# salesforce/ai-economist

Measured on AMD Instinct MI355X. Metric: agent-steps/sec, gather-trade-build 25x25 4-agent batched envs, higher is better.
Workload: dtype u8/i32 state + f64 coin/utility (f32 observations); 1 GPU; C2 BASELINE configs[1]: gather-trade-build 25x25, 4 agents + planner, Build+CDA+Gather+PeriodicBracketTax, 4096 replicas/GPU, uniform random policy, planner not counted; envs_per_gpu=4096, global_envs=4096, n_agents=4, kernel_specialisation=compile time, parallelism=single GPU

## Files before the change

### ai-economist_amd/csrc/aie_capi.hip

```cpp
#include <hip/hip_runtime.h>

#include <cstdio>
#include <cstdlib>
#include <cstring>
#include <vector>

#include "aie_kernels.hip"
#include "aie_kernels_sampler.hip"
#include "aie_kernels_rollout.hip"
#include "aie_kernels_ose.hip"
#include "aie_kernels_saez.hip"
#include "aie_kernels_ppo.hip"
#include "aie_kernels_mlp.hip"
#include "aie_kernels_mlp_bwd.hip"
#include "aie_kernels_covid.hip"
#include "aie_jit.h"
#include "aie_layout_build.h"
#include "aie_trainer_plan.h"

struct aie_env {
  aie_params P{};
  aie_params* d_params;
  aie_tensor_table tt;
  uint8_t* arena;
// ... 73 lines not shown
        for (size_t q = 0; q < off; q += piece) (void)hipMemUnmap(static_cast<char*>(va) + q, piece);
        (void)hipMemAddressFree(va, total);
      }
    }
    (void)hipGetLastError();
  }
  return hipMalloc(&p, bytes) == hipSuccess ? static_cast<uint8_t*>(p) : nullptr;
}
static void aie_arena_free(uint8_t* arena, size_t vmm_total, size_t vmm_piece) {
  if (!arena) return;
  if (vmm_total) {
    for (size_t q = 0; q < vmm_total; q += vmm_piece) (void)hipMemUnmap(arena + q, vmm_piece);
    (void)hipMemAddressFree(arena, vmm_total);
  } else {
    (void)hipFree(arena);
  }
}

__global__ void aie_init_cells_kernel(const aie_params P, uint8_t* __restrict__ arena) {
  const int64_t q = (int64_t)blockIdx.x * blockDim.x + threadIdx.x;
  if (q >= (int64_t)P.E * P.HW) return;
  const int e = (int)(q / P.HW), cell = (int)(q - (int64_t)e * P.HW);
  reinterpret_cast<uint32_t*>(arena + P.a_records + (int64_t)e * P.rec_bytes + P.o_cells)[cell] = 0x00ff0000u;
}

__global__ void aie_set_flags_kernel(const aie_params P, uint8_t* __restrict__ arena,
                                     const uint8_t* __restrict__ flags, int shared) {
  const int64_t q = (int64_t)blockIdx.x * blockDim.x + threadIdx.x;
  if (q >= (int64_t)P.E * P.HW) return;
  const int e = (int)(q / P.HW), cell = (int)(q - (int64_t)e * P.HW);
  uint32_t* w = reinterpret_cast<uint32_t*>(arena + P.a_records + (int64_t)e * P.rec_bytes + P.o_cells) + cell;
  const uint32_t fl = flags[shared ? cell : q];
  *w = (*w & 0x00ffffffu) | (fl << 24);
}

__global__ void __launch_bounds__(64) aie_src_list_kernel(const aie_params* __restrict__ params, uint8_t* __restrict__ arena) {
  const aie_params& P = *params;
  const int e = (int)blockIdx.x, lane = (int)threadIdx.x, HW = P.HW;
  if (!P.o_src_list || e >= P.E) return;
  uint8_t* rec = arena + P.a_records + (int64_t)e * P.rec_bytes;
  const uint8_t* cb = rec + P.o_cells;
  uint16_t* lst = reinterpret_cast<uint16_t*>(rec + P.o_src_list);
  for (int k = lane; k < AIE_SRC_CAP; k += 64) lst[k] = 0;
  int base = 0;
  for (int rs = 0; rs < 2; ++rs) {
    const uint32_t bit = rs == 0 ? AIE_CELL_WOOD_SRC : AIE_CELL_STONE_SRC;
    for (int q0 = 0; q0 < HW; q0 += 64) {
      const int q = q0 + lane;
      const bool on = q < HW && (cb[4 * q + 3] & bit);
      const uint64_t mask = __ballot(on);
      const int slot = base + __popcll(mask & ((1ull << lane) - 1ull));
      if (on && slot < AIE_SRC_CAP) lst[slot] = (uint16_t)(rs * HW + q);
      base += __popcll(mask);
    }
  }
  if (lane == 0) *reinterpret_cast<int32_t*>(rec + P.o_src_n) = base;
}
static int aie_rebuild_src_lists(aie_env* env) {
  if (env->P.c.scenario != AIE_SCN_GTB || !env->P.o_src_list) return AIE_OK;
  hipLaunchKernelGGL(aie_src_list_kernel, dim3((unsigned)env->P.E), dim3(64), 0, 0, env->d_params, env->arena);
  AIE_HIP_CHECK(env, hipGetLastError());
  AIE_HIP_CHECK(env, hipDeviceSynchronize());
  return AIE_OK;
}

static inline int aie_workgroups_per_cu(size_t lds) {
// ... 1008 lines not shown
```

### ai-economist_amd/csrc/aie_gtb_state.h

```cpp
#pragma once
#include "aie_device.h"

namespace aie {
__device__ __forceinline__ bool can_agent_occupy(const Ctx& c, int r, int col, int agent) {
  if (r < 0 || r >= c.P.H || col < 0 || col >= c.P.W) return false;
  const int cell = r * c.P.W + col;
  const uint32_t w = R_CELLS(c)[cell];
  if (AIE_CELL_FLAGS(w) & AIE_CELL_WATER) return false;
  const int o = AIE_CELL_OWNER(w);
  if (!(o < 0 || o == agent)) return false;
  const int occ = c.locmap[cell];
  return occ == 0 || occ == agent + 1;
}

__device__ __forceinline__ void log_event(const Ctx& c, int type, int a1, int a2, int a3, int a4, int a5,
                                          int a6, int a7, int a8, double f) {
  if (c.tid != 0) return;
  const int k = c.srcn[2];
  if (k >= c.R.ev_cap) return;
  int32_t* row = c.ev + 4 + k * AIE_EV_WORDS;
  row[0] = type; row[1] = a1; row[2] = a2; row[3] = a3; row[4] = a4;
  row[5] = a5; row[6] = a6; row[7] = a7; row[8] = a8; row[9] = 0;
  *reinterpret_cast<double*>(row + 10) = f;
  c.srcn[2] = k + 1;
// ... 121 lines not shown
        if (x >= x0 && x < x0 + P.n_sub_p * P.sub_p_dim && (x - x0) / P.sub_p_dim == i) v = (x - x0) % P.sub_p_dim + 1;
      }
    }
    c.act_p[i] = v;
  }
  if (host && P.n_host_p && ap && i < P.n_host_p) {
    const int32_t* a = ap + (int64_t)c.e * P.act_p_width;
    int v;
    if (P.c.multi_action_mode_planner) {
      v = a[P.hp_row[i]];
      if (v < 0 || v > P.hp_dim[i]) { bad_p = true; v = 0; }
    } else {
      const int x = a[0];
      if (x < 0 || x >= P.AP) bad_p = true;
      v = (x >= P.hp_base[i] && x < P.hp_base[i] + P.hp_dim[i]) ? x - P.hp_base[i] + 1 : 0;
    }
    reinterpret_cast<int32_t*>(arena + c.R.a_host_act_p)[(int64_t)c.e * P.n_host_p + i] = v;
  }
  return (__ballot(bad_a) ? AIE_ERR_AGENT_ACTION : 0) | (__ballot(bad_p) ? AIE_ERR_PLANNER_ACTION : 0);
}

__device__ __forceinline__ uint16_t* dirty_list(const Ctx& c) { return reinterpret_cast<uint16_t*>(c.dirty + 4); }
__device__ __forceinline__ void dirty_add_uniform(const Ctx& c, MTL& m, int cell) {
  if (c.tid == 0 && m.dn < AIE_DIRTY_CAP) dirty_list(c)[m.dn] = (uint16_t)cell;
  m.dn += 1;
}
__device__ __forceinline__ void dirty_add_lane(const Ctx& c, int cell) {
  const int s = atomicAdd(&c.dirty[0], 1);
  if (s < AIE_DIRTY_CAP) dirty_list(c)[s] = (uint16_t)cell;
}
__device__ __forceinline__ void dirty_agent_moved(MTL& m, int i) {
  if (i < 32) m.mv0 |= 1u << i; else m.mv1 |= 1u << (i - 32);
}
__device__ __forceinline__ void store_record_step(const Ctx& c, uint8_t* __restrict__ arena, int wave, int nwaves) {
  uint8_t* g = arena + (int64_t)c.e * c.P.rec_bytes;
  uint4* dst = reinterpret_cast<uint4*>(g);
  const uint4* src = reinterpret_cast<const uint4*>(c.rec);
  const int nq = rec_lds_bytes(c.P) >> 4;
  const int cnt = uni(c.dirty[0]);
  const int q0 = (c.P.o_cells == 0 && cnt <= AIE_DIRTY_CAP) ? (4 * c.P.HW) >> 4 : 0;
  for (int q = q0 + wave * AIE_NT + c.tid; q < nq; q += nwaves * AIE_NT) dst[q] = src[q];
  if (wave == nwaves - 1 && q0 > 0 && c.tid < cnt) {
    const int cell = (int)dirty_list(c)[c.tid];
    reinterpret_cast<uint32_t*>(g + c.P.o_cells)[cell] = R_CELLS(c)[cell];
  }
}

}
```

### ai-economist_amd/csrc/aie_kernels.hip

```cpp
#pragma once
#include "aie_gtb_state.h"
#include "aie_gtb_components.h"
#include "aie_gtb_observe.h"
#include "aie_gtb_layoutgen.h"



__device__ __forceinline__ uint32_t glibc_tables_touch(int lane) {
  uint32_t v = 0;
#pragma unroll
  for (int k = 0; k < 2; ++k) {
    const int line = 2 * lane + k;
    const uint8_t* p = line < 48 ? reinterpret_cast<const uint8_t*>(aie_glibc_powlog_tab) + 64 * line
                     : line < 80 ? reinterpret_cast<const uint8_t*>(aie_glibc_exp_tab) + 64 * (line - 48)
                                 : reinterpret_cast<const uint8_t*>(aie_glibc_log_tab) + 64 * (line - 80);
    if (line < 112) v ^= *reinterpret_cast<const volatile uint32_t*>(p);
  }
  return v;
}

__device__ __forceinline__ void step_rewards_and_done(const aie::Ctx& c, uint8_t* __restrict__ arena, const NextActions& next, int skip,
                                                      bool emit = true, bool close = true) {
  using namespace aie;
  float* const rew_log = close ? rew_log_claim(c.R, R_I32(c, o_rew_slot), R_I32(c, o_rew_epoch), c.R.E, c.P.n, c.tid == 0) : nullptr;
// ... 27 lines not shown
#endif
  const int e_blk = replica_of_block((int)blockIdx.x, next.E);
  if (next.e_hi > 0 && (e_blk < next.e_lo || e_blk >= next.e_hi)) return;
  if (LOG && next.mask && !next.mask[e_blk]) return;
  const bool FAST = rng_fast(P);
  const int tid0 = (int)(threadIdx.x & (AIE_NT - 1));
  uint8_t* grec = arena + (int64_t)e_blk * P.rec_bytes;
  uint32_t* gkey = reinterpret_cast<uint32_t*>(grec + P.o_mt);
  const Ctx c = make_ctx(P, R, lds, e_blk, tid0, arena, LOG, skip,
                         SPEC >= 0);
  const bool SHL = shared_src_list(P);
  uint32_t* const draw_w = reinterpret_cast<uint32_t*>(c.stage);
  int draw_cap = stage_window_words(P);
  if (LOG && R.dev_draw_window > 0 && R.dev_draw_window < draw_cap) draw_cap = R.dev_draw_window;
  const int w0_tail_prio = P.n >= 8 ? 2 : 0;
  const bool REW_ON_W1 = FAST && P.n < 8;
  const int ph = LOG ? next.phase : 0;
  const bool HEAD = ph == 0 || (ph & 1), TAIL = ph == 0 || (ph & 2), OBSERVE = ph != 0 && (ph & 4) && !(ph & 2);
  const bool REBASE = OBSERVE && (ph & 8);
  const bool RETAX = OBSERVE && (ph & 16);
  const bool REGEN = TAIL || (ph & 64), EMIT = TAIL || (ph & 128), CLOSE = TAIL || (ph & 256);
  const bool CLOSE_ONLY = CLOSE && !EMIT;
  const int c_lo = ph ? next.comp_lo : 0, c_hi = ph ? next.comp_hi : P.c.n_components;
  constexpr int COMP_UNROLL = (SPEC >= 0 && !LOG) ? AIE_MAX_COMPONENTS : 1;
  if (wid == 0) {
    Agents A;
    A.hist_dirty = 0;
    A.tax_dirty = false;
    int act_err = 0;
    if (!(skip & AIE_DEV_SKIP_ACTION_DECODE)) act_err = decode_actions(c, A, act_a, act_p, arena);
    else A.act = 0;
    if (TRACE && R.dev_trace && c.tid == 0) R.dev_trace[12 * blockIdx.x] = wall_clock64();
    if (TRACE && R.dev_trace && c.tid == 0) R.dev_trace[12 * blockIdx.x + 9] = wall_clock64();
    MT none;
    load_record(c, arena, none, 0, 2, -1);
    __syncthreads();
    if (TRACE && R.dev_trace && c.tid == 0) R.dev_trace[12 * blockIdx.x + 8] = wall_clock64();
    MTL ml{draw_w, 0, 0u, -AIE_MT_N, 0, 0u, 0u, 0, 0, 0, FAST ? reinterpret_cast<uint32_t*>(c.rec + P.o_mt) : gkey, draw_cap, FAST};
    ml.pos = ml.base = uni(*R_I32(c, o_mt_pos));
    ml.avail = ml.cap < AIE_MT_N - ml.pos ? ml.cap : AIE_MT_N - ml.pos;
    if (FAST) {
      const int covered = 128 * ((ml.cap + 127) >> 7) - (ml.pos & 1);
      if (ml.avail > covered) ml.avail = covered;
    }
    agents_load(c, A);
#ifdef AIE_FLAT_FULL
    const bool flat_in_place = false;
#else
    const bool flat_in_place = ph == 0 && uni(*R_I32(c, o_obs_valid)) != 0 && !(skip & AIE_DEV_FLAT_FULL);
#endif
    if (act_err && c.tid == 0) *R_I32(c, o_error_flags) |= act_err;
    bool cda_in_range = ph == 0;
    if (ph != 0)
      for (int k = c_lo; k < c_hi; ++k) cda_in_range |= P.c.components[k] == AIE_COMP_CDA;
    if (P.has_cda && !(skip & AIE_DEV_SKIP_COMPONENTS) && cda_in_range) cda_decay_price_history(c);
    __syncthreads();
    if (c.tid == 0 && HEAD) *R_I32(c, o_timestep) += 1;
    if (c.ev && c.tid == 0) c.srcn[2] = 0;
    __builtin_amdgcn_s_setprio(3);
    if (TRACE && R.dev_trace && c.tid == 0) R.dev_trace[12 * blockIdx.x + 1] = wall_clock64();
    if (!(skip & AIE_DEV_SKIP_COMPONENTS)) {
#pragma unroll COMP_UNROLL
      for (int k = c_lo; k < c_hi; ++k) {
        switch (P.c.components[k]) {
          case AIE_COMP_BUILD: if (!(skip & AIE_DEV_SKIP_BUILD)) build_component_step(c, ml, A); break;
          case AIE_COMP_CDA: if (!(skip & AIE_DEV_SKIP_CDA)) cda_component_step(c, A); break;
          case AIE_COMP_GATHER: if (!(skip & AIE_DEV_SKIP_GATHER)) gather_component_step(c, ml, A); break;
          case AIE_COMP_TAX: if (!(skip & AIE_DEV_SKIP_TAX)) tax_component_step(c, ml, A); break;
          case AIE_COMP_WEALTH_REDISTRIBUTION: wealth_component_step(c, A); break;
          default: break;
        }
// ... 9 lines not shown
      c.dirty[1] = (int32_t)ml.mv0;
      c.dirty[2] = (int32_t)ml.mv1;
      c.dirty[3] = ml.tw;
    }
    if (TRACE && R.dev_trace && c.tid == 0) R.dev_trace[12 * blockIdx.x + 5] = wall_clock64();
    __syncthreads();
    if (w0_tail_prio) __builtin_amdgcn_s_setprio(2);
    if (RETAX && P.has_tax) {
      if (c.tid < P.n) R_F64(c, o_tax_last_coin)[c.tid] = R_F64(c, o_inv_coin)[c.tid] + R_F64(c, o_esc_coin)[c.tid];
      AIE_WSYNC();
    }
    if (!(skip & AIE_DEV_SKIP_FLAT_AND_MASKS) && (EMIT || OBSERVE)) {
      const bool annealed_first = P.has_tax && P.c.tax_annealing && uni(*R_I32(c, o_timestep)) == 1;
      if (flat_in_place && !A.tax_dirty && !annealed_first) update_flat_observations(c, arena, A.hist_dirty);
      else write_flat_observations(c, arena);
    }
    if (TRACE && R.dev_trace && c.tid == 0) R.dev_trace[12 * blockIdx.x + 10] = wall_clock64();
    if (!REW_ON_W1 && (EMIT || CLOSE)) step_rewards_and_done(c, arena, next, skip, EMIT, CLOSE);
    if (REBASE) {
      AIE_WSYNC();
      current_metrics(c);
      AIE_WSYNC();
      if (c.tid <= P.n) R_F64(c, o_util)[c.tid] = scr_part(c)[c.tid];
      AIE_WSYNC();
    }
    if (w0_tail_prio) __builtin_amdgcn_s_setprio(0);
    __syncthreads();
    if (!(skip & AIE_DEV_SKIP_RECORD_STORE)) store_record_step(c, arena, 0, 2);
    if (TRACE && R.dev_trace && c.tid == 0) R.dev_trace[12 * blockIdx.x + 7] = wall_clock64();
  } else {
    MT m;
    mt_init(m, P);
    const int gpos = *reinterpret_cast<const int32_t*>(grec + P.o_mt_pos);
    load_record(c, arena, m, 1, 2, -1);
    if (skip & AIE_DEV_SKIP_DRAW_WINDOW) {}
    else if (FAST) draw_window_publish_fast(draw_w, draw_cap, (uint32_t)uni((int)gkey[0]), (uint32_t)uni((int)gkey[1]), (uint32_t)uni((int)gkey[2]), uni(gpos), c.tid);
    else draw_window_publish_from_hbm(draw_w, draw_cap, gkey, uni(gpos), c.tid);

    if (SPEC >= 0 && const_tables_in_lds(P)) {
      if (P.has_tax && P.c.tax_model == AIE_TAX_MODEL_WRAPPER)
        for (int q = c.tid; q < P.c.tax_n_disc_rates; q += AIE_NT) const_cast<double*>(c.rtab)[q] = R.c.tax_disc_rates[q];
      for (int q = c.tid; q < P.MA; q += AIE_NT) const_cast<uint32_t*>(c.mtab)[q] = P.mask_test[q];
    }
    __syncthreads();
    if (!(skip & AIE_DEV_SKIP_LOCMAP)) rebuild_locmap(c);
    __syncthreads();
    SrcList src;
    src.S = 0;
#pragma unroll
    for (int k = 0; k < AIE_SRC_CAP / AIE_NT; ++k) src.d[k] = 0;
    src = SHL ? src_list_from_arena(c, arena) : src_list_from_record(c, arena);
    const uint32_t warm = glibc_tables_touch(c.tid);
    if (!FAST && !(skip & AIE_DEV_SKIP_GENERATOR_ROWS)) {
#pragma unroll
      for (int j = 0; j < 9; ++j) m.r[j] = gkey[64 * j + c.tid];
      m.r[9] = c.tid < 48 ? gkey[576 + c.tid] : 0u;
    }
    if ((next.a || next.p) && TAIL) {
      const int per_env = P.n * P.act_a_width + P.act_p_width;
      const int st = uni(*R_I32(c, o_sample_t));
      for (int j = c.tid; j < per_env; j += AIE_NT) sample_action_slot(P, next.seed, next.env_offset, (int64_t)st, c.e, j, next.a, next.p);
      if (c.tid == 0) *R_I32(c, o_sample_t) = st + 1;
    }
    asm volatile("" ::"v"(warm));
    __syncthreads();
    if (next.E > 6144) __builtin_amdgcn_s_setprio(0);
    else __builtin_amdgcn_s_setprio(2);
    if (FAST) {
      const uint32_t* st = R_U32(c, o_mt);
      m.fkey = (uint32_t)uni((int)st[0]);
      m.fblk = (uint32_t)uni((int)st[1]);
      m.fsalt = (uint32_t)uni((int)st[2]);
    } else if (uni(c.dirty[3]) != 0) {
      mt_rows_from_hbm(m, gkey, c.tid);
    }
    m.pos = uni(*R_I32(c, o_mt_pos));
    if (REGEN) {
// ... 269 lines not shown
        if (++tries > 200) {
          *R_I32(c, o_error_flags) |= AIE_ERR_RESET_PLACEMENT;
          break;
        }
      }
      R_I32(c, o_loc_r)[i] = r;
      R_I32(c, o_loc_c)[i] = col;
      c.locmap[r * P.W + col] = (uint8_t)(i + 1);
    }
  }
  *R_I32(c, o_mt_pos) = m.pos;
  mt_fast_detach(c, m);
  __syncthreads();
  current_metrics(c);
  __syncthreads();
  if (tid <= n) R_F64(c, o_util)[tid] = scr_part(c)[tid];
  __syncthreads();
  write_spatial_observations(c, arena);
  if (tid == 0) *R_I32(c, o_obs_valid) = 1;
  write_flat_observations(c, arena);
  AIE_WSYNC();
  if (P.has_tax && P.c.tax_annealing && tid == 0) *R_I32(c, o_tax_last_completions) = *R_I32(c, o_completions);
  AIE_WSYNC();
  write_action_masks(c, arena);
  if (!keep_rewards) {
    if (tid < n) reinterpret_cast<float*>(arena + R.a_rew_a)[(int64_t)e * n + tid] = 0.0f;
    if (tid == 0) {
      reinterpret_cast<float*>(arena + R.a_rew_p)[e] = 0.0f;
      (arena + R.a_done)[e] = 0;
    }
  }
  __syncthreads();
  store_record(c, arena, m);
}
}

#ifndef AIE_JIT
extern "C" __global__ void __launch_bounds__(AIE_NT)
aie_reset_kernel(const aie_params* __restrict__ params, uint8_t* __restrict__ arena,
                 const uint8_t* __restrict__ mask, int keep_rewards) {
  extern __shared__ __attribute__((aligned(16))) uint8_t lds[];
  aie::reset_body<-1, false>(params, arena, mask, keep_rewards, lds);
}
extern "C" __global__ void __launch_bounds__(LG_NW * AIE_NT)
aie_reset_kernel_layout(const aie_params* __restrict__ params, uint8_t* __restrict__ arena,
                        const uint8_t* __restrict__ mask, int keep_rewards) {
  extern __shared__ __attribute__((aligned(16))) uint8_t lds[];
  aie::reset_body<-1, true>(params, arena, mask, keep_rewards, lds);
}
extern "C" __global__ void aie_layout_decide_kernel(const aie_params* __restrict__ params, uint8_t* __restrict__ arena, int threshold) {
  int32_t* ctl = reinterpret_cast<int32_t*>(arena + params->a_layout_ctl);
  const bool go = ctl[0] >= threshold;
  ctl[1] = go ? 1 : 0;
  if (go) ctl[0] = 0;
}
extern "C" __global__ void __launch_bounds__(LG_NW * AIE_NT)
aie_layout_refill_kernel(const aie_params* __restrict__ params, uint8_t* __restrict__ arena) {
  extern __shared__ __attribute__((aligned(16))) uint8_t lds[];
  const aie_params& P = *params;
  const int32_t* ctl = reinterpret_cast<const int32_t*>(arena + P.a_layout_ctl);
  if (!ctl[1]) return;
  const int e = (int)blockIdx.x, gtid = (int)threadIdx.x;
  const uint32_t* stg = reinterpret_cast<const uint32_t*>(arena + P.a_records + (int64_t)e * P.rec_bytes + P.o_mt);
  uint32_t st[4];
#pragma unroll
  for (int k = 0; k < 4; ++k) st[k] = (uint32_t)aie::uni((int)stg[k]);
// ... 91 lines not shown
```

### ai-economist_amd/csrc/aie_layout.h

```cpp
#ifndef AIE_LAYOUT_H_
#define AIE_LAYOUT_H_

#include <math.h>
#include <stdio.h>
#include <string.h>

#include "aie.h"

#if defined(__HIPCC__)
#define AIE_HD __host__ __device__
#else
#define AIE_HD
#endif

#define AIE_MAX_TENSORS 160
#define AIE_MAX_MASK 544

enum {
  AIE_SUB_BUILD = 0,
  AIE_SUB_BUY0 = 1,
  AIE_SUB_SELL0 = 2,
  AIE_SUB_BUY1 = 3,
  AIE_SUB_SELL1 = 4,
  AIE_SUB_GATHER = 5,
// ... 77 lines not shown
  int32_t o_inv_coin, o_esc_coin, o_labor, o_build_payment, o_build_skill, o_bonus_gather_prob;
  int32_t o_util;
  int32_t o_cda_n_bids, o_cda_n_asks, o_cda_bids, o_cda_asks, o_cda_n_orders;
  int32_t o_cda_bid_hist, o_cda_ask_hist, o_cda_price_history;
  int32_t o_tax_cycle_pos, o_tax_rate_idx, o_tax_last_coin, o_tax_last_income;
  int32_t o_tax_last_marginal_rate, o_tax_total_collected;
  int32_t o_timestep, o_completions, o_auto_warmup;
  int32_t o_mask_bits, o_mask_p_open;
  int32_t o_skill, o_production, o_first_step;
  int32_t o_mt, o_mt_pos, o_mt_has_gauss, o_mt_gauss;
  int32_t o_tax_last_completions;
  int32_t o_error_flags;
  int32_t o_src_n, o_src_list;
  int32_t o_obs_valid;

  int64_t a_records;
  int64_t a_obs_a_map, a_obs_a_idx, a_obs_a_flat, a_obs_a_mask, a_obs_a_time;
  int64_t a_obs_p_map, a_obs_p_idx, a_obs_p_flat, a_obs_p_mask, a_obs_p_time, a_obs_p_agents;
  int64_t a_rew_a, a_rew_p, a_done;
  int64_t arena_bytes;

  uint32_t mg_WV2, mg_WV, mg_MA, mg_FA, mg_P, mg_2P, mg_taxA, mg_HW, mg_W, mg_sub_p, mg_sub_p_dim;

  int32_t regen_conv;
  int32_t regen_general;
  int32_t o_regen_count;
  double regen_p[AIE_N_RES][50];
  int64_t a_saez;
  int32_t saez_stride, saez_cap;
  int64_t a_saez_global;
  int32_t saez_global_cap, saez_pad_;
  int64_t a_layout_prob;
  int64_t a_layout_stage, a_layout_tag, a_layout_ctl;
  int32_t layout_stage_stride, layout_pad_;
  int64_t a_src_list;
  int32_t o_tax_saez_rates;
  int32_t o_tax_saez_obs_rates;
  double saez_edges[AIE_SAEZ_BINS + 1];
  int64_t a_events;
  int32_t ev_replicas, ev_cap, ev_stride, ev_pad_;
  int64_t a_metrics;
  int32_t met_bytes;
  int32_t mo_cda;
  int32_t mo_tax_sched;
  int32_t mo_tax_income;
  int32_t mo_tax_paid;
  int32_t mo_tax_eff;
  int32_t mo_tax_occ;
  int32_t mo_tax_days;
  uint32_t mask_test[AIE_MAX_MASK];
  int32_t dev_skip_mask;
  uint64_t* dev_trace;
  float* rew_log;
  int32_t rew_slots, rew_epoch;

  int32_t cv_L;
  int32_t cv_F;
  int32_t cv_NL;
  int32_t cv_NS;
  int32_t cv_nch;
  int32_t cv_row;
  int32_t cv_nrow_obs;
  int32_t cv_pitch;
  int32_t cv_t_first_delivery;
  int32_t o_cv_state;
  int32_t o_cv_cooldown;
  int32_t o_cv_subsidy_level;
// ... 103 lines not shown
#define AIE_FA_TAX_LEN(NB, n) ((NB) + (n) + 4)
#define AIE_FP_TAX_PHASE(NB, n) ((NB) + 2 + (n))
#define AIE_FP_TAX_LEN(NB, n) ((NB) + (n) + 3)
enum { AIE_FPA_TAX_CURR_MARGINAL_RATE = 0, AIE_FPA_TAX_LAST_INCOME = 1, AIE_FPA_TAX_LAST_MARGINAL_RATE = 2, AIE_FPA_TAX_LEN = 3 };

static inline uint32_t aie__magic(int64_t d) {
  return d <= 1 ? 0u : (uint32_t)((0x100000000ll + d - 1) / d);
}

static inline int64_t aie__align(int64_t x, int64_t a) { return (x + a - 1) / a * a; }

static inline int aie__dtype_size(int dt) {
  switch (dt) {
    case AIE_U8: case AIE_I8: return 1;
    case AIE_I16: return 2;
    case AIE_I32: case AIE_U32: case AIE_F32: return 4;
    default: return 8;
  }
}

static inline int aie__has(const aie_config* c, int comp) {
  for (int i = 0; i < c->n_components; ++i)
    if (c->components[i] == comp) return 1;
  return 0;
}

#define AIE_SRC_CAP 128
static inline int aie__shared_src_list(const aie_config* c) {
  return c->scenario == AIE_SCN_GTB && c->shared_layout && c->layout_gen == AIE_LAYOUT_FIXED;
}
static inline int aie__record_src_list(const aie_config* c) {
  return c->scenario == AIE_SCN_GTB && !(aie__shared_src_list(c) && c->rng_mode == AIE_RNG_FAST);
}
static inline int32_t aie__rng_state_words(const aie_config* c) { return c->rng_mode == AIE_RNG_FAST ? 4 : AIE_MT_N; }
AIE_HD static inline int aie__layout_staged(const aie_config* c) {
  return c->scenario == AIE_SCN_GTB && c->layout_gen != AIE_LAYOUT_FIXED && c->rng_mode == AIE_RNG_FAST;
}
AIE_HD static inline void aie_layout_stream(const uint32_t st[4], uint32_t out[2]) {
  out[0] = st[0] + 0x9E3779B9u * (st[3] >> 15);
  out[1] = st[2] | 0x8000u | (st[3] & 0x7fffu);
}
AIE_HD static inline uint64_t aie_layout_tag(const uint32_t st[4]) {
  uint32_t ks[2];
  aie_layout_stream(st, ks);
  return ((uint64_t)ks[0] << 32) | (uint64_t)ks[1];
}

enum {
  AIE_CV_K_POP = 0, AIE_CV_K_BETA_SLOPE, AIE_CV_K_BETA_INTERCEPT, AIE_CV_K_UNEMP_BIAS,
  AIE_CV_K_MAX_PROD, AIE_CV_K_HEALTH_NORM, AIE_CV_K_ECON_NORM,
  AIE_CV_K_MIN_HEALTH, AIE_CV_K_MAX_HEALTH, AIE_CV_K_MIN_ECON, AIE_CV_K_MAX_ECON,
  AIE_CV_K_W_HEALTH, AIE_CV_K_W_ECON, AIE_CV_K_MAX_DAILY_SUBSIDY, AIE_CV_K_VACCINES_PER_DELIVERY,
  AIE_CV_K_S0, AIE_CV_K_I0, AIE_CV_K_R0, AIE_CV_K_D0, AIE_CV_K_U0, AIE_CV_K_V0,
  AIE_CV_K_CONV_W0,
  AIE_CV_K_COUNT = AIE_CV_K_CONV_W0 + AIE_COVID_MAX_FILTERS
};
enum { AIE_CV_ST_S = 0, AIE_CV_ST_I, AIE_CV_ST_R, AIE_CV_ST_D, AIE_CV_ST_V, AIE_CV_ST_U,
       AIE_CV_ST_PROD, AIE_CV_ST_SUBSIDY,
       AIE_CV_ST_HEALTH_INDEX, AIE_CV_ST_ECONOMIC_INDEX,
       AIE_CV_ST_COUNT };
enum { AIE_CV_SUM_UNEMPLOYED = 0, AIE_CV_SUM_STRINGENCY, AIE_CV_SUM_PRODUCTIVITY, AIE_CV_SUM_SUBSIDY, AIE_CV_SUM_COUNT };
enum { AIE_CV_OB_STATE = 0, AIE_CV_OB_PROD = 6, AIE_CV_OB_LAG = 7, AIE_CV_OB_TIME = 8, AIE_CV_OB_POLICY = 9,
       AIE_CV_OB_T_SUBSIDY = 10, AIE_CV_OB_SUBSIDY_LEVEL = 11, AIE_CV_OB_T_VACCINE = 12, AIE_CV_OB_MASK = 13 };

#define AIE_CV_GROUP 2
#define AIE_CV_EVENT_CAP 64
// ... 5 lines not shown

#define AIE_SAEZ_OFF_ELAS 16
#define AIE_SAEZ_OFF_AVG (AIE_SAEZ_OFF_ELAS + 32)
#define AIE_SAEZ_OFF_NEXT (AIE_SAEZ_OFF_AVG + 8 * AIE_MAX_BRACKETS)
#define AIE_SAEZ_OFF_BUF (AIE_SAEZ_OFF_NEXT + 8 * AIE_MAX_BRACKETS)

AIE_HD static inline uint32_t aie_counter_rng(uint64_t seed, uint64_t env, uint64_t t, uint64_t slot) {
  uint64_t z = seed + 0x9E3779B97F4A7C15ull * (env + 1ull);
  z ^= (t + 1ull) * 0xBF58476D1CE4E5B9ull;
  z ^= (slot + 1ull) * 0x94D049BB133111EBull;
  z = (z ^ (z >> 30)) * 0xBF58476D1CE4E5B9ull;
  z = (z ^ (z >> 27)) * 0x94D049BB133111EBull;
  z ^= z >> 31;
  return (uint32_t)(z >> 32);
}

AIE_HD static inline double aie_annealed_tax_limit(int completions, double warmup, double slope, double final_max) {
  double pv = slope * ((double)completions - warmup);
  pv = pv < 1.0 ? pv : 1.0;
  pv = pv > 0.0 ? pv : 0.0;
  return pv * final_max;
}

#define AIE_CELL_WATER 1u
#define AIE_CELL_STONE_SRC 2u
#define AIE_CELL_WOOD_SRC 4u
#define AIE_CELL_STONE(w) ((w) & 0xffu)
#define AIE_CELL_WOOD(w) (((w) >> 8) & 0xffu)
#define AIE_CELL_OWNER(w) ((int)(int8_t)(((w) >> 16) & 0xffu))
#define AIE_CELL_FLAGS(w) (((w) >> 24) & 0xffu)
#define AIE_CELL_PACK(st, wd, own, fl) \
  ((uint32_t)(st) | ((uint32_t)(wd) << 8) | (((uint32_t)(own) & 0xffu) << 16) | ((uint32_t)(fl) << 24))

#define AIE_ORD_AGENT(o) ((o) & 0xff)
#define AIE_ORD_PRICE(o) (((o) >> 8) & 0xff)
#define AIE_ORD_LIFE(o) (((o) >> 16) & 0xffff)
#define AIE_ORD_PACK(a, p, l) ((int32_t)((a) | ((p) << 8) | ((l) << 16)))

#if !defined(__HIPCC__) && !defined(AIE_LAYOUT_H_ONLY)
#include "aie_layout_build.h"
#include "aie_trainer_math.h"
#endif

#endif
```

### ai-economist_amd/csrc/aie_layout_build.h

```cpp
#ifndef AIE_LAYOUT_BUILD_H_
#define AIE_LAYOUT_BUILD_H_

#include <stdio.h>
#include <string.h>

#ifndef AIE_LAYOUT_H_ONLY
#define AIE_LAYOUT_H_ONLY 1
#endif
#include "aie_layout.h"

typedef struct aie_tensor_table {
  int32_t n;
  aie_tensor_desc t[AIE_MAX_TENSORS];
} aie_tensor_table;

#define AIE__FAIL(...)                                   \
  do {                                                   \
    if (err) snprintf(err, errlen, __VA_ARGS__);         \
    return AIE_E_INVALID;                                \
  } while (0)

static inline int32_t aie__rec(int32_t* cur, int32_t bytes, int32_t align) {
  int32_t o = (int32_t)aie__align(*cur, align);
  *cur = o + bytes;
// ... 762 lines not shown
  }
  if (p->has_tax) {
    p->o_tax_last_coin = aie__rec(&cur, 8 * n, 8);
    p->o_tax_last_income = aie__rec(&cur, 8 * n, 8);
    p->o_tax_last_marginal_rate = aie__rec(&cur, 8 * n, 8);
    p->o_tax_total_collected = aie__rec(&cur, 8, 8);
    p->o_tax_cycle_pos = aie__rec(&cur, 4, 4);
    p->o_tax_last_completions = aie__rec(&cur, 4, 4);
    p->o_tax_rate_idx = aie__rec(&cur, 4 * p->NB, 4);
    if (c->tax_model == AIE_TAX_SAEZ) {
      p->o_tax_saez_rates = aie__rec(&cur, 8 * p->NB, 8);
      p->o_tax_saez_obs_rates = aie__rec(&cur, 8 * p->NB, 8);
    }
  }
  p->o_timestep = aie__rec(&cur, 4, 4);
  p->o_completions = aie__rec(&cur, 4, 4);
  p->o_auto_warmup = aie__rec(&cur, 4, 4);
  p->o_obs_valid = aie__rec(&cur, 4, 4);
  p->o_error_flags = aie__rec(&cur, 4, 4);
  p->o_sample_t = aie__rec(&cur, 4, 4);
  p->o_rew_slot = aie__rec(&cur, 4, 4);
  p->o_rew_epoch = aie__rec(&cur, 4, 4);
  p->o_mask_bits = aie__rec(&cur, 4 * n, 4);
  p->o_mask_p_open = aie__rec(&cur, 4, 4);
  p->o_mt_gauss = aie__rec(&cur, 8, 8);
  p->o_mt_pos = aie__rec(&cur, 4, 4);
  p->o_mt_has_gauss = aie__rec(&cur, 4, 4);
  p->o_mt = aie__rec(&cur, 4 * aie__rng_state_words(c), 16);
  p->o_src_n = p->o_src_list = 0;
  if (aie__record_src_list(c)) {
    p->o_src_n = aie__rec(&cur, 16, 16);
    p->o_src_list = aie__rec(&cur, 2 * AIE_SRC_CAP, 16);
  }
  p->rec_bytes = (int32_t)aie__align(cur, 16);

  const int64_t E = p->E;
  int64_t a = 0;
  p->a_records = a; a = aie__align(a + E * (int64_t)p->rec_bytes, 256);
  p->am_ch = c->full_observability ? p->CM : p->CM + 1;
  p->am_h = c->full_observability ? p->H : p->WV;
  p->am_w = c->full_observability ? p->W : p->WV;
  const int64_t wv2 = (int64_t)p->am_h * p->am_w;
  p->a_obs_a_map = a;  a = aie__align(a + E * n * p->am_ch * wv2 * 4, 256);
  p->a_obs_a_idx = a;  a = aie__align(a + E * n * 2 * wv2 * 2, 256);
  p->a_obs_a_flat = a; a = aie__align(a + E * n * p->FA * 4, 256);
  p->a_obs_a_mask = a; a = aie__align(a + E * n * p->MA * 4, 256);
  p->a_obs_a_time = a; a = aie__align(a + E * n * 4, 256);
  if (c->planner_gets_spatial_info) {
    p->a_obs_p_map = a; a = aie__align(a + E * p->CM * HW * 4, 256);
    p->a_obs_p_idx = a; a = aie__align(a + E * 2 * HW * 2, 256);
  }
  p->a_obs_p_flat = a;   a = aie__align(a + E * p->FP * 4, 256);
  p->a_obs_p_mask = a;   a = aie__align(a + E * p->MP * 4, 256);
  p->a_obs_p_time = a;   a = aie__align(a + E * 4, 256);
  p->a_obs_p_agents = a; a = aie__align(a + E * n * (p->FPA ? p->FPA : 1) * 4, 256);
  p->a_rew_a = a; a = aie__align(a + E * n * 4, 256);
  p->a_rew_p = a; a = aie__align(a + E * 4, 256);
  p->a_done = a;  a = aie__align(a + E, 256);
  aie__alloc_metrics(p, &a);
  aie__alloc_events(c, p, &a);
  aie__alloc_saez(c, p, &a);
  p->a_layout_prob = a;
  if (c->layout_gen != AIE_LAYOUT_FIXED) a = aie__align(a + (int64_t)AIE_N_RES * HW * 8, 256);
  p->layout_stage_stride = (HW + 15) / 16 * 16;
  p->layout_pad_ = 0;
  p->a_layout_stage = p->a_layout_tag = p->a_layout_ctl = a;
  if (aie__layout_staged(c)) {
    p->a_layout_stage = a; a = aie__align(a + E * p->layout_stage_stride, 256);
    p->a_layout_tag = a;   a = aie__align(a + E * 8, 256);
    p->a_layout_ctl = a;   a = aie__align(a + 16, 256);
  }
  p->a_src_list = a;
  if (aie__shared_src_list(c)) a = aie__align(a + 16 + 2 * AIE_SRC_CAP, 256);
  p->a_host_act_a = p->a_host_act_p = a;
  if (p->n_host_a) { p->a_host_act_a = a; a = aie__align(a + E * n * p->n_host_a * 4, 256); }
  if (p->n_host_p) { p->a_host_act_p = a; a = aie__align(a + E * p->n_host_p * 4, 256); }
  p->arena_bytes = a;

  if (tt) {
    const int64_t rs = p->rec_bytes, r0 = p->a_records;
#define REC(name, dt, off, nd, d0, d1, d2) aie__add(tt, name, dt, r0 + (off), rs, nd, d0, d1, d2, 0, E)
    REC("cells", AIE_U32, p->o_cells, 2, p->H, p->W, 0);
    {
      static const char* nm[4] = {"stone", "wood", "house_owner", "cell_flags"};
      for (int b = 0; b < 4; ++b) {
        REC(nm[b], b == 2 ? AIE_I8 : AIE_U8, p->o_cells + b, 2, p->H, p->W, 0);
        aie_tensor_desc* d = &tt->t[tt->n - 1];
        d->stride[2] = 4;
        d->stride[1] = 4 * (int64_t)p->W;
      }
    }
    if (p->regen_conv) REC("regen_source_count", AIE_U8, p->o_regen_count, 3, R, p->H, p->W);
    REC("loc_r", AIE_I32, p->o_loc_r, 1, n, 0, 0);
    REC("loc_c", AIE_I32, p->o_loc_c, 1, n, 0, 0);
    REC("inv_res", AIE_I32, p->o_inv_res, 2, R, n, 0);
    REC("esc_res", AIE_I32, p->o_esc_res, 2, R, n, 0);
    REC("inv_coin", AIE_F64, p->o_inv_coin, 1, n, 0, 0);
    REC("esc_coin", AIE_F64, p->o_esc_coin, 1, n, 0, 0);
// ... 6 lines not shown
      REC("cda_n_bids", AIE_I32, p->o_cda_n_bids, 1, R, 0, 0);
      REC("cda_n_asks", AIE_I32, p->o_cda_n_asks, 1, R, 0, 0);
      REC("cda_bids", AIE_I32, p->o_cda_bids, 2, R, p->M, 0);
      REC("cda_asks", AIE_I32, p->o_cda_asks, 2, R, p->M, 0);
      REC("cda_n_orders", AIE_I32, p->o_cda_n_orders, 2, R, n, 0);
      REC("cda_bid_hist", AIE_U8, p->o_cda_bid_hist, 3, R, n, p->P);
      REC("cda_ask_hist", AIE_U8, p->o_cda_ask_hist, 3, R, n, p->P);
      REC("cda_price_history", AIE_F64, p->o_cda_price_history, 3, R, n, p->P);
    }
    if (p->has_tax) {
      REC("tax_cycle_pos", AIE_I32, p->o_tax_cycle_pos, 0, 0, 0, 0);
    REC("tax_last_completions", AIE_I32, p->o_tax_last_completions, 0, 0, 0, 0);
      REC("tax_rate_idx", AIE_I32, p->o_tax_rate_idx, 1, p->NB, 0, 0);
      if (c->tax_model == AIE_TAX_SAEZ) {
        REC("tax_saez_bracket_rates", AIE_F64, p->o_tax_saez_rates, 1, p->NB, 0, 0);
        REC("tax_saez_observed_rates", AIE_F64, p->o_tax_saez_obs_rates, 1, p->NB, 0, 0);
      }
      REC("tax_last_coin", AIE_F64, p->o_tax_last_coin, 1, n, 0, 0);
      REC("tax_last_income", AIE_F64, p->o_tax_last_income, 1, n, 0, 0);
      REC("tax_last_marginal_rate", AIE_F64, p->o_tax_last_marginal_rate, 1, n, 0, 0);
      REC("tax_total_collected", AIE_F64, p->o_tax_total_collected, 0, 0, 0, 0);
    }
    REC("timestep", AIE_I32, p->o_timestep, 0, 0, 0, 0);
    REC("completions", AIE_I32, p->o_completions, 0, 0, 0, 0);
    REC("sample_t", AIE_I32, p->o_sample_t, 0, 0, 0, 0);
    REC("rew_log_slot", AIE_I32, p->o_rew_slot, 0, 0, 0, 0);
    REC("auto_warmup", AIE_I32, p->o_auto_warmup, 0, 0, 0, 0);
    REC("obs_valid", AIE_I32, p->o_obs_valid, 0, 0, 0, 0);
    REC("error_flags", AIE_I32, p->o_error_flags, 0, 0, 0, 0);
    if (p->o_src_list) {
      REC("regen_src_n", AIE_I32, p->o_src_n, 0, 0, 0, 0);
      REC("regen_src_list", AIE_I16, p->o_src_list, 1, AIE_SRC_CAP, 0, 0);
    }
    REC("mt", AIE_U32, p->o_mt, 1, aie__rng_state_words(&p->c), 0, 0);
    REC("mt_pos", AIE_I32, p->o_mt_pos, 0, 0, 0, 0);
    REC("mt_has_gauss", AIE_I32, p->o_mt_has_gauss, 0, 0, 0, 0);
    REC("mt_gauss", AIE_F64, p->o_mt_gauss, 0, 0, 0, 0);
#undef REC
#define DENSE(name, dt, off, nd, d0, d1, d2, d3)                                            \
  do {                                                                                      \
    int64_t dd[4] = {d0, d1, d2, d3};                                                       \
    int64_t es = aie__dtype_size(dt);                                                       \
    for (int q = 0; q < nd; ++q) es *= dd[q];                                               \
    aie__add(tt, name, dt, off, es, nd, d0, d1, d2, d3, E);                                 \
  } while (0)
    DENSE("obs_a_world-map", AIE_F32, p->a_obs_a_map, 4, n, p->am_ch, p->am_h, p->am_w);
    DENSE("obs_a_world-idx_map", AIE_I16, p->a_obs_a_idx, 4, n, 2, p->am_h, p->am_w);
    DENSE("obs_a_flat", AIE_F32, p->a_obs_a_flat, 2, n, p->FA, 0, 0);
    DENSE("obs_a_action_mask", AIE_F32, p->a_obs_a_mask, 2, n, p->MA, 0, 0);
    DENSE("obs_a_time", AIE_F32, p->a_obs_a_time, 2, n, 1, 0, 0);
    if (c->planner_gets_spatial_info) {
      DENSE("obs_p_world-map", AIE_F32, p->a_obs_p_map, 3, p->CM, p->H, p->W, 0);
      DENSE("obs_p_world-idx_map", AIE_I16, p->a_obs_p_idx, 3, 2, p->H, p->W, 0);
    }
    DENSE("obs_p_flat", AIE_F32, p->a_obs_p_flat, 1, p->FP, 0, 0, 0);
    DENSE("obs_p_action_mask", AIE_F32, p->a_obs_p_mask, 1, p->MP, 0, 0, 0);
    DENSE("obs_p_time", AIE_F32, p->a_obs_p_time, 1, 1, 0, 0, 0);
    if (p->FPA) DENSE("obs_p_agents", AIE_F32, p->a_obs_p_agents, 2, n, p->FPA, 0, 0);
    DENSE("rewards_a", AIE_F32, p->a_rew_a, 1, n, 0, 0, 0);
    DENSE("rewards_p", AIE_F32, p->a_rew_p, 0, 0, 0, 0, 0);
    DENSE("done", AIE_U8, p->a_done, 0, 0, 0, 0, 0);
    aie__add_metrics_tensors(p, tt);
    aie__add_event_tensors(p, tt);
    aie__add_saez_tensors(p, tt);
    if (c->layout_gen != AIE_LAYOUT_FIXED)
      aie__add_shared(tt, "layout_source_prob", AIE_F64, p->a_layout_prob, 2, AIE_N_RES, HW);
// ... 10 lines not shown
```

### ai-economist_amd/csrc/aie_spec_generated.h

```cpp
#pragma once
#define AIE_N_SPECS 9
template <int K> struct aie_spec_image;
alignas(16) static constexpr unsigned char aie_spec_bytes_0[8824] = {
  11,0,0,0,0,0,0,0,4,0,0,0,25,0,0,0,25,0,0,0,90,90,90,90,0,0,0,0,1,0,0,0,
  1,0,0,0,4,0,0,0,1,0,0,0,2,0,0,0,3,0,0,0,4,0,0,0,0,0,0,0,0,0,0,0,
  0,0,0,0,0,0,0,0,1,0,0,0,1,0,0,0,1,0,0,0,0,0,0,0,5,0,0,0,0,0,0,0,
  0,0,0,0,0,0,0,0,0,0,0,0,0,0,0,0,0,0,0,0,1,0,0,0,1,0,0,0,0,0,0,0,
  90,90,90,90,90,90,90,90,90,90,90,90,90,90,90,90,90,90,90,90,90,90,90,90,90,90,90,90,90,90,90,90,
  90,90,90,90,90,90,90,90,90,90,90,90,90,90,90,90,90,90,90,90,90,90,90,90,90,90,90,90,90,90,90,90,
  90,90,90,90,90,90,90,90,90,90,90,90,90,90,90,90,90,90,90,90,90,90,90,90,90,90,90,90,90,90,90,90,
  90,90,90,90,90,90,90,90,90,90,90,90,90,90,90,90,90,90,90,90,90,90,90,90,90,90,90,90,90,90,90,90,
  90,90,90,90,90,90,90,90,90,90,90,90,90,90,90,90,90,90,90,90,90,90,90,90,90,90,90,90,90,90,90,90,
  90,90,90,90,90,90,90,90,90,90,90,90,90,90,90,90,90,90,90,90,90,90,90,90,90,90,90,90,90,90,90,90,
  90,90,90,90,90,90,90,90,90,90,90,90,90,90,90,90,90,90,90,90,90,90,90,90,90,90,90,90,90,90,90,90,
  90,90,90,90,90,90,90,90,90,90,90,90,90,90,90,90,90,90,90,90,90,90,90,90,90,90,90,90,90,90,90,90,
  90,90,90,90,90,90,90,90,90,90,90,90,90,90,90,90,90,90,90,90,90,90,90,90,90,90,90,90,90,90,90,90,
  90,90,90,90,90,90,90,90,90,90,90,90,90,90,90,90,90,90,90,90,90,90,90,90,90,90,90,90,90,90,90,90,
  90,90,90,90,90,90,90,90,90,90,90,90,90,90,90,90,90,90,90,90,90,90,90,90,90,90,90,90,90,90,90,90,
  90,90,90,90,90,90,90,90,90,90,90,90,90,90,90,90,90,90,90,90,90,90,90,90,90,90,90,90,90,90,90,90,
  90,90,90,90,90,90,90,90,90,90,90,90,90,90,90,90,90,90,90,90,90,90,90,90,90,90,90,90,90,90,90,90,
  90,90,90,90,90,90,90,90,90,90,90,90,90,90,90,90,90,90,90,90,90,90,90,90,90,90,90,90,90,90,90,90,
  90,90,90,90,90,90,90,90,90,90,90,90,90,90,90,90,90,90,90,90,90,90,90,90,90,90,90,90,90,90,90,90,
  90,90,90,90,90,90,90,90,90,90,90,90,90,90,90,90,90,90,90,90,90,90,90,90,90,90,90,90,90,90,90,90,
  90,90,90,90,90,90,90,90,90,90,90,90,90,90,90,90,90,90,90,90,90,90,90,90,90,90,90,90,90,90,90,90,
// ... 74 lines not shown
  0,0,0,0,0,0,0,0,0,0,0,0,0,0,0,0,0,0,0,0,0,0,0,0,0,0,0,0,0,0,0,0,
  0,0,0,0,0,0,0,0,0,0,0,0,0,0,0,0,0,0,0,0,0,0,0,0,0,0,0,0,0,0,0,0,
  0,0,0,0,0,0,0,0,0,0,0,0,0,0,0,0,0,0,0,0,0,0,0,0,0,0,0,0,0,0,0,0,
  0,0,0,0,0,0,0,0,0,0,0,0,0,0,0,0,0,0,0,0,0,0,0,0,0,0,0,0,0,0,0,0,
  0,0,0,0,0,0,0,0,0,0,0,0,0,0,0,0,0,0,0,0,0,0,0,0,0,0,0,0,0,0,0,0,
  0,0,0,0,0,0,0,0,0,0,0,0,0,0,0,0,0,0,0,0,0,0,0,0,0,0,0,0,0,0,0,0,
  0,0,0,0,0,0,0,0,0,0,0,0,0,0,0,0,0,0,0,0,0,0,0,0,0,0,0,0,0,0,0,0,
  0,0,0,0,0,0,0,0,0,0,0,0,0,0,0,0,0,0,0,0,0,0,0,0,0,0,0,0,0,0,0,0,
  0,0,0,0,0,0,0,0,0,0,0,0,0,0,0,0,0,0,0,0,0,0,0,0,0,0,0,0,0,0,0,0,
  0,0,0,0,0,0,0,0,0,0,0,0,0,0,0,0,0,0,0,0,0,0,0,0,0,0,0,0,0,0,0,0,
  0,0,0,0,0,0,0,0,0,0,0,0,0,0,0,0,0,0,0,0,0,0,0,0,0,0,0,0,0,0,0,0,
  0,0,0,0,0,0,0,0,0,0,0,0,0,0,0,0,0,0,0,0,0,0,0,0,0,0,0,0,0,0,0,0,
  0,0,0,0,0,0,0,0,0,0,0,0,0,0,0,0,0,0,0,0,0,0,0,0,0,0,0,0,90,90,90,90,
  90,90,90,90,0,0,0,0,0,0,0,0,0,0,0,0,90,90,90,90,90,90,90,90,90,90,90,90,90,90,90,90,
  90,90,90,90,90,90,90,90,90,90,90,90,90,90,90,90,90,90,90,90,0,0,0,0,0,0,0,0,0,0,0,0,
  90,90,90,90,90,90,90,90,0,0,0,0,0,0,0,0,90,90,90,90,90,90,90,90,90,90,90,90,90,90,90,90,
  90,90,90,90,90,90,90,90,90,90,90,90,90,90,90,90,0,0,0,0,0,0,0,0,0,0,0,0,0,0,0,0,
  0,0,0,0,0,0,0,0,0,0,0,0,0,0,0,0,0,0,0,0,0,0,0,0,0,0,0,0,0,0,0,0,
  0,0,0,0,0,0,0,0,0,0,0,0,0,0,0,0,0,0,0,0,0,0,0,0,0,0,0,0,0,0,0,0,
  0,0,0,0,0,0,0,0,0,0,0,0,0,0,0,0,0,0,0,0,0,0,0,0,0,0,0,0,0,0,0,0,
  0,0,0,0,0,0,0,0,0,0,0,0,0,0,0,0,0,0,0,0,0,0,0,0,0,0,0,0,0,0,0,0,
  0,0,0,0,0,0,0,0,0,0,0,0,0,0,0,0,0,0,0,0,4,0,0,0,25,0,0,0,25,0,0,0,
  113,2,0,0,11,0,0,0,7,0,0,0,20,0,0,0,6,0,0,0,11,0,0,0,7,0,0,0,11,0,0,0,
  11,0,0,0,1,0,0,0,1,0,0,0,1,0,0,0,1,0,0,0,0,0,0,0,1,0,0,0,6,0,0,0,
  0,0,0,0,1,0,0,0,2,0,0,0,3,0,0,0,4,0,0,0,5,0,0,0,0,0,0,0,0,0,0,0,
  0,0,0,0,0,0,0,0,0,0,0,0,0,0,0,0,0,0,0,0,0,0,0,0,0,0,0,0,0,0,0,0,
  1,0,0,0,11,0,0,0,11,0,0,0,11,0,0,0,11,0,0,0,4,0,0,0,0,0,0,0,0,0,0,0,
  0,0,0,0,0,0,0,0,0,0,0,0,0,0,0,0,0,0,0,0,0,0,0,0,0,0,0,0,0,0,0,0,
  1,0,0,0,2,0,0,0,13,0,0,0,24,0,0,0,35,0,0,0,46,0,0,0,0,0,0,0,0,0,0,0,
  0,0,0,0,0,0,0,0,0,0,0,0,0,0,0,0,0,0,0,0,0,0,0,0,0,0,0,0,0,0,0,0,
  50,0,0,0,7,0,0,0,21,0,0,0,148,0,0,0,21,0,0,0,1,0,0,0,7,0,0,0,136,0,0,0,
  86,0,0,0,8,0,0,0,0,0,0,0,2,0,0,0,114,0,0,0,115,0,0,0,130,0,0,0,131,0,0,0,
  0,0,0,0,68,0,0,0,82,0,0,0,83,0,0,0,0,0,0,0,3,0,0,0,0,0,0,0,50,0,0,0,
  154,0,0,0,144,27,0,0,0,0,0,0,176,10,0,0,192,10,0,0,208,10,0,0,240,10,0,0,200,9,0,0,
  232,9,0,0,8,10,0,0,40,10,0,0,72,10,0,0,104,10,0,0,136,10,0,0,208,13,0,0,216,13,0,0,
  224,13,0,0,128,14,0,0,32,15,0,0,64,15,0,0,152,15,0,0,16,11,0,0,88,16,0,0,96,16,0,0,
  240,15,0,0,16,16,0,0,48,16,0,0,80,16,0,0,124,16,0,0,128,16,0,0,132,16,0,0,156,16,0,0,
  172,16,0,0,0,0,0,0,0,0,0,0,0,0,0,0,192,16,0,0,184,16,0,0,188,16,0,0,176,16,0,0,
  92,16,0,0,140,16,0,0,128,26,0,0,144,26,0,0,136,16,0,0,0,0,0,0,0,0,0,0,0,0,0,0,
  0,0,0,0,0,0,0,0,0,0,0,0,0,0,0,0,0,0,0,0,0,0,0,0,0,0,0,0,0,0,0,0,
  0,0,0,0,0,0,0,0,0,0,0,0,0,0,0,0,0,0,0,0,0,0,0,0,0,0,0,0,0,0,0,0,
  0,0,0,0,0,0,0,0,0,0,0,0,0,0,0,0,0,0,0,0,0,0,0,0,0,0,0,0,0,0,0,0,
  0,0,0,0,0,0,0,0,0,0,0,0,0,0,0,0,0,0,0,0,0,0,0,0,174,158,29,2,117,209,69,23,
  82,184,30,5,226,225,225,1,117,209,69,23,187,232,162,11,18,17,17,17,140,219,104,0,164,112,61,10,187,232,162,11,
  13,195,48,12,0,0,0,0,0,0,0,0,0,0,0,0,90,90,90,90,90,90,90,90,90,90,90,90,90,90,90,90,
  90,90,90,90,90,90,90,90,90,90,90,90,90,90,90,90,90,90,90,90,90,90,90,90,90,90,90,90,90,90,90,90,
  90,90,90,90,90,90,90,90,90,90,90,90,90,90,90,90,90,90,90,90,90,90,90,90,90,90,90,90,90,90,90,90,
  90,90,90,90,90,90,90,90,90,90,90,90,90,90,90,90,90,90,90,90,90,90,90,90,90,90,90,90,90,90,90,90,
  90,90,90,90,90,90,90,90,90,90,90,90,90,90,90,90,90,90,90,90,90,90,90,90,90,90,90,90,90,90,90,90,
  90,90,90,90,90,90,90,90,90,90,90,90,90,90,90,90,90,90,90,90,90,90,90,90,90,90,90,90,90,90,90,90,
  90,90,90,90,90,90,90,90,90,90,90,90,90,90,90,90,90,90,90,90,90,90,90,90,90,90,90,90,90,90,90,90,
  90,90,90,90,90,90,90,90,90,90,90,90,90,90,90,90,90,90,90,90,90,90,90,90,90,90,90,90,90,90,90,90,
  90,90,90,90,90,90,90,90,90,90,90,90,90,90,90,90,90,90,90,90,90,90,90,90,90,90,90,90,90,90,90,90,
  90,90,90,90,90,90,90,90,90,90,90,90,90,90,90,90,90,90,90,90,90,90,90,90,90,90,90,90,90,90,90,90,
  90,90,90,90,90,90,90,90,90,90,90,90,90,90,90,90,90,90,90,90,90,90,90,90,90,90,90,90,90,90,90,90,
  90,90,90,90,90,90,90,90,90,90,90,90,90,90,90,90,90,90,90,90,90,90,90,90,90,90,90,90,90,90,90,90,
  90,90,90,90,90,90,90,90,90,90,90,90,90,90,90,90,90,90,90,90,90,90,90,90,90,90,90,90,90,90,90,90,
  90,90,90,90,90,90,90,90,90,90,90,90,90,90,90,90,90,90,90,90,90,90,90,90,90,90,90,90,90,90,90,90,
  90,90,90,90,90,90,90,90,90,90,90,90,90,90,90,90,90,90,90,90,90,90,90,90,90,90,90,90,90,90,90,90,
  90,90,90,90,90,90,90,90,90,90,90,90,90,90,90,90,90,90,90,90,90,90,90,90,90,90,90,90,90,90,90,90,
  90,90,90,90,90,90,90,90,90,90,90,90,90,90,90,90,90,90,90,90,90,90,90,90,90,90,90,90,90,90,90,90,
  90,90,90,90,90,90,90,90,90,90,90,90,90,90,90,90,90,90,90,90,90,90,90,90,90,90,90,90,90,90,90,90,
  90,90,90,90,90,90,90,90,90,90,90,90,90,90,90,90,90,90,90,90,90,90,90,90,90,90,90,90,90,90,90,90,
  90,90,90,90,90,90,90,90,90,90,90,90,90,90,90,90,90,90,90,90,90,90,90,90,90,90,90,90,90,90,90,90,
  90,90,90,90,90,90,90,90,90,90,90,90,90,90,90,90,90,90,90,90,90,90,90,90,90,90,90,90,90,90,90,90,
  90,90,90,90,90,90,90,90,90,90,90,90,90,90,90,90,90,90,90,90,90,90,90,90,90,90,90,90,90,90,90,90,
  90,90,90,90,90,90,90,90,90,90,90,90,90,90,90,90,90,90,90,90,90,90,90,90,90,90,90,90,90,90,90,90,
  90,90,90,90,90,90,90,90,90,90,90,90,90,90,90,90,90,90,90,90,90,90,90,90,90,90,90,90,90,90,90,90,
  90,90,90,90,90,90,90,90,90,90,90,90,90,90,90,90,90,90,90,90,90,90,90,90,90,90,90,90,90,90,90,90,
  90,90,90,90,90,90,90,90,90,90,90,90,90,90,90,90,0,0,0,0,0,0,0,0,0,0,0,0,0,0,0,0,
  0,0,0,0,0,0,0,0,0,0,0,0,0,0,0,0,0,0,0,0,0,0,0,0,0,0,0,0,0,0,0,0,
  0,0,0,0,0,0,0,0,0,0,0,0,0,0,0,0,128,2,0,0,0,0,0,0,0,0,0,0,0,0,0,0,
  0,0,0,0,0,0,0,0,90,90,90,90,90,90,90,90,90,90,90,90,90,90,90,90,90,90,90,90,90,90,90,90,
  90,90,90,90,90,90,90,90,90,90,90,90,90,90,90,90,90,90,90,90,90,90,90,90,90,90,90,90,90,90,90,90,
  90,90,90,90,90,90,90,90,90,90,90,90,90,90,90,90,90,90,90,90,90,90,90,90,90,90,90,90,90,90,90,90,
  90,90,90,90,90,90,90,90,90,90,90,90,90,90,90,90,90,90,90,90,90,90,90,90,90,90,90,90,90,90,90,90,
  90,90,90,90,90,90,90,90,90,90,90,90,90,90,90,90,90,90,90,90,90,90,90,90,90,90,90,90,90,90,90,90,
  90,90,90,90,90,90,90,90,90,90,90,90,90,90,90,90,90,90,90,90,90,90,90,90,90,90,90,90,90,90,90,90,
  90,90,90,90,90,90,90,90,90,90,90,90,90,90,90,90,90,90,90,90,90,90,90,90,90,90,90,90,90,90,90,90,
  90,90,90,90,90,90,90,90,90,90,90,90,90,90,90,90,90,90,90,90,90,90,90,90,90,90,90,90,90,90,90,90,
  90,90,90,90,90,90,90,90,90,90,90,90,90,90,90,90,90,90,90,90,90,90,90,90,90,90,90,90,90,90,90,90,
  90,90,90,90,90,90,90,90,90,90,90,90,90,90,90,90,90,90,90,90,90,90,90,90,90,90,90,90,90,90,90,90,
  90,90,90,90,90,90,90,90,90,90,90,90,90,90,90,90,90,90,90,90,90,90,90,90,90,90,90,90,90,90,90,90,
  90,90,90,90,90,90,90,90,90,90,90,90,90,90,90,90,90,90,90,90,90,90,90,90,90,90,90,90,90,90,90,90,
  90,90,90,90,90,90,90,90,90,90,90,90,90,90,90,90,90,90,90,90,90,90,90,90,90,90,90,90,90,90,90,90,
  90,90,90,90,90,90,90,90,90,90,90,90,90,90,90,90,90,90,90,90,90,90,90,90,90,90,90,90,90,90,90,90,
  90,90,90,90,90,90,90,90,90,90,90,90,90,90,90,90,90,90,90,90,90,90,90,90,90,90,90,90,90,90,90,90,
  90,90,90,90,90,90,90,90,90,90,90,90,90,90,90,90,90,90,90,90,90,90,90,90,90,90,90,90,90,90,90,90,
  90,90,90,90,90,90,90,90,90,90,90,90,90,90,90,90,90,90,90,90,90,90,90,90,90,90,90,90,90,90,90,90,
  90,90,90,90,90,90,90,90,90,90,90,90,90,90,90,90,90,90,90,90,90,90,90,90,90,90,90,90,90,90,90,90,
  90,90,90,90,90,90,90,90,90,90,90,90,90,90,90,90,90,90,90,90,90,90,90,90,90,90,90,90,90,90,90,90,
  90,90,90,90,90,90,90,90,90,90,90,90,90,90,90,90,90,90,90,90,90,90,90,90,90,90,90,90,90,90,90,90,
  90,90,90,90,90,90,90,90,90,90,90,90,90,90,90,90,90,90,90,90,90,90,90,90,90,90,90,90,90,90,90,90,
  90,90,90,90,90,90,90,90,90,90,90,90,90,90,90,90,90,90,90,90,90,90,90,90,90,90,90,90,90,90,90,90,
  90,90,90,90,90,90,90,90,90,90,90,90,90,90,90,90,90,90,90,90,90,90,90,90,90,90,90,90,90,90,90,90,
  90,90,90,90,90,90,90,90,90,90,90,90,90,90,90,90,90,90,90,90,90,90,90,90,90,90,90,90,90,90,90,90,
  90,90,90,90,90,90,90,90,90,90,90,90,90,90,90,90,90,90,90,90,90,90,90,90,90,90,90,90,90,90,90,90,
  90,90,90,90,90,90,90,90,90,90,90,90,90,90,90,90,0,0,0,0,0,0,0,0,0,0,0,0,0,0,0,0,
  0,0,0,0,0,0,0,0,0,0,0,0,0,0,0,0,32,1,0,0,128,0,0,0,0,0,0,0,56,0,0,0,
  88,0,0,0,120,0,0,0,0,1,0,0,28,1,0,0,0,0,0,0,0,1,1,0,8,255,1,0,8,255,2,0,
  8,255,3,0,8,255,4,0,8,255,5,0,8,255,6,0,8,255,7,0,8,255,8,0,8,255,9,0,8,255,10,0,
  8,255,11,0,5,1,1,0,5,1,1,0,5,1,1,0,5,1,1,0,5,1,1,0,5,1,1,0,5,1,1,0,
  5,1,1,0,5,1,1,0,5,1,1,0,5,1,1,0,16,255,1,0,16,255,2,0,16,255,3,0,16,255,4,0,
  16,255,5,0,16,255,6,0,16,255,7,0,16,255,8,0,16,255,9,0,16,255,10,0,16,255,11,0,6,1,1,0,
  6,1,1,0,6,1,1,0,6,1,1,0,6,1,1,0,6,1,1,0,6,1,1,0,6,1,1,0,6,1,1,0,
// ... 732 lines not shown
  0,0,0,0,0,0,0,0,0,0,0,0,0,0,0,0,0,0,0,0,0,0,0,0,0,0,0,0,0,0,0,0,
  0,0,0,0,0,0,0,0,0,0,0,0,0,0,0,0,0,0,0,0,0,0,0,0,0,0,0,0,0,0,0,0,
  0,0,0,0,0,0,0,0,0,0,0,0,0,0,0,0,0,0,0,0,0,0,0,0,0,0,0,0,0,0,0,0,
  0,0,0,0,0,0,0,0,0,0,0,0,0,0,0,0,0,0,0,0,0,0,0,0,0,0,0,0,0,0,0,0,
  0,0,0,0,0,0,0,0,0,0,0,0,0,0,0,0,0,0,0,0,0,0,0,0,0,0,0,0,0,0,0,0,
  0,0,0,0,0,0,0,0,0,0,0,0,0,0,0,0,0,0,0,0,0,0,0,0,0,0,0,0,0,0,0,0,
  0,0,0,0,0,0,0,0,0,0,0,0,0,0,0,0,0,0,0,0,0,0,0,0,0,0,0,0,0,0,0,0,
  0,0,0,0,0,0,0,0,0,0,0,0,0,0,0,0,0,0,0,0,0,0,0,0,0,0,0,0,0,0,0,0,
  0,0,0,0,0,0,0,0,0,0,0,0,0,0,0,0,0,0,0,0,0,0,0,0,0,0,0,0,0,0,0,0,
  0,0,0,0,0,0,0,0,0,0,0,0,0,0,0,0,0,0,0,0,0,0,0,0,0,0,0,0,0,0,0,0,
  0,0,0,0,0,0,0,0,0,0,0,0,0,0,0,0,0,0,0,0,0,0,0,0,0,0,0,0,0,0,0,0,
  0,0,0,0,0,0,0,0,0,0,0,0,0,0,0,0,0,0,0,0,0,0,0,0,0,0,0,0,0,0,0,0,
  0,0,0,0,0,0,0,0,0,0,0,0,0,0,0,0,0,0,0,0,0,0,0,0,0,0,0,0,90,90,90,90,
  90,90,90,90,0,0,0,0,0,0,0,0,0,0,0,0,90,90,90,90,90,90,90,90,90,90,90,90,90,90,90,90,
  90,90,90,90,90,90,90,90,90,90,90,90,90,90,90,90,90,90,90,90,0,0,0,0,0,0,0,0,0,0,0,0,
  90,90,90,90,90,90,90,90,1,0,0,0,0,0,0,0,90,90,90,90,90,90,90,90,90,90,90,90,90,90,90,90,
  90,90,90,90,90,90,90,90,90,90,90,90,90,90,90,90,0,0,0,0,0,0,0,0,0,0,0,0,0,0,0,0,
  0,0,0,0,0,0,0,0,0,0,0,0,0,0,0,0,0,0,0,0,0,0,0,0,0,0,0,0,0,0,0,0,
  0,0,0,0,0,0,0,0,0,0,0,0,0,0,0,0,0,0,0,0,0,0,0,0,0,0,0,0,0,0,0,0,
  0,0,0,0,0,0,0,0,0,0,0,0,0,0,0,0,0,0,0,0,0,0,0,0,0,0,0,0,0,0,0,0,
  0,0,0,0,0,0,0,0,0,0,0,0,0,0,0,0,0,0,0,0,0,0,0,0,0,0,0,0,0,0,0,0,
  0,0,0,0,0,0,0,0,0,0,0,0,0,0,0,0,0,0,0,0,4,0,0,0,15,0,0,0,15,0,0,0,
  225,0,0,0,0,0,0,0,0,0,0,0,0,0,0,0,5,0,0,0,11,0,0,0,6,0,0,0,11,0,0,0,
  11,0,0,0,1,0,0,0,0,0,0,0,1,0,0,0,0,0,0,0,0,0,0,0,0,0,0,0,2,0,0,0,
  0,0,0,0,5,0,0,0,0,0,0,0,0,0,0,0,0,0,0,0,0,0,0,0,0,0,0,0,0,0,0,0,
  0,0,0,0,0,0,0,0,0,0,0,0,0,0,0,0,0,0,0,0,0,0,0,0,0,0,0,0,0,0,0,0,
  1,0,0,0,4,0,0,0,0,0,0,0,0,0,0,0,0,0,0,0,0,0,0,0,0,0,0,0,0,0,0,0,
  0,0,0,0,0,0,0,0,0,0,0,0,0,0,0,0,0,0,0,0,0,0,0,0,0,0,0,0,0,0,0,0,
  1,0,0,0,2,0,0,0,0,0,0,0,0,0,0,0,0,0,0,0,0,0,0,0,0,0,0,0,0,0,0,0,
  0,0,0,0,0,0,0,0,0,0,0,0,0,0,0,0,0,0,0,0,0,0,0,0,0,0,0,0,0,0,0,0,
  6,0,0,0,0,0,0,0,0,0,0,0,1,0,0,0,0,0,0,0,1,0,0,0,1,0,0,0,9,0,0,0,
  4,0,0,0,5,0,0,0,0,0,0,0,2,0,0,0,2,0,0,0,3,0,0,0,3,0,0,0,4,0,0,0,
  0,0,0,0,0,0,0,0,0,0,0,0,1,0,0,0,0,0,0,0,0,0,0,0,0,0,0,0,6,0,0,0,
  1,0,0,0,240,15,0,0,0,0,0,0,112,4,0,0,128,4,0,0,144,4,0,0,176,4,0,0,136,3,0,0,
  168,3,0,0,200,3,0,0,232,3,0,0,8,4,0,0,40,4,0,0,72,4,0,0,0,0,0,0,0,0,0,0,
  0,0,0,0,0,0,0,0,0,0,0,0,0,0,0,0,0,0,0,0,0,0,0,0,0,0,0,0,0,0,0,0,
  0,0,0,0,0,0,0,0,0,0,0,0,0,0,0,0,208,4,0,0,212,4,0,0,216,4,0,0,240,4,0,0,
  0,5,0,0,0,0,0,0,0,0,0,0,0,0,0,0,32,5,0,0,16,5,0,0,20,5,0,0,8,5,0,0,
  0,0,0,0,224,4,0,0,224,14,0,0,240,14,0,0,220,4,0,0,0,0,0,0,0,0,0,0,0,0,0,0,
  0,0,0,0,0,0,0,0,0,0,0,0,0,0,0,0,0,0,0,0,0,0,0,0,0,0,0,0,0,0,0,0,
  0,0,0,0,0,0,0,0,0,0,0,0,0,0,0,0,0,0,0,0,0,0,0,0,0,0,0,0,0,0,0,0,
  0,0,0,0,0,0,0,0,0,0,0,0,0,0,0,0,0,0,0,0,0,0,0,0,0,0,0,0,0,0,0,0,
  0,0,0,0,0,0,0,0,0,0,0,0,0,0,0,0,0,0,0,0,0,0,0,0,174,158,29,2,117,209,69,23,
  171,170,170,42,29,199,113,28,0,0,0,0,0,0,0,0,0,0,0,32,104,69,35,1,18,17,17,17,0,0,0,0,
  0,0,0,0,0,0,0,0,0,0,0,0,0,0,0,0,90,90,90,90,90,90,90,90,90,90,90,90,90,90,90,90,
  90,90,90,90,90,90,90,90,90,90,90,90,90,90,90,90,90,90,90,90,90,90,90,90,90,90,90,90,90,90,90,90,
  90,90,90,90,90,90,90,90,90,90,90,90,90,90,90,90,90,90,90,90,90,90,90,90,90,90,90,90,90,90,90,90,
  90,90,90,90,90,90,90,90,90,90,90,90,90,90,90,90,90,90,90,90,90,90,90,90,90,90,90,90,90,90,90,90,
  90,90,90,90,90,90,90,90,90,90,90,90,90,90,90,90,90,90,90,90,90,90,90,90,90,90,90,90,90,90,90,90,
  90,90,90,90,90,90,90,90,90,90,90,90,90,90,90,90,90,90,90,90,90,90,90,90,90,90,90,90,90,90,90,90,
  90,90,90,90,90,90,90,90,90,90,90,90,90,90,90,90,90,90,90,90,90,90,90,90,90,90,90,90,90,90,90,90,
  90,90,90,90,90,90,90,90,90,90,90,90,90,90,90,90,90,90,90,90,90,90,90,90,90,90,90,90,90,90,90,90,
  90,90,90,90,90,90,90,90,90,90,90,90,90,90,90,90,90,90,90,90,90,90,90,90,90,90,90,90,90,90,90,90,
  90,90,90,90,90,90,90,90,90,90,90,90,90,90,90,90,90,90,90,90,90,90,90,90,90,90,90,90,90,90,90,90,
  90,90,90,90,90,90,90,90,90,90,90,90,90,90,90,90,90,90,90,90,90,90,90,90,90,90,90,90,90,90,90,90,
  90,90,90,90,90,90,90,90,90,90,90,90,90,90,90,90,90,90,90,90,90,90,90,90,90,90,90,90,90,90,90,90,
  90,90,90,90,90,90,90,90,90,90,90,90,90,90,90,90,90,90,90,90,90,90,90,90,90,90,90,90,90,90,90,90,
  90,90,90,90,90,90,90,90,90,90,90,90,90,90,90,90,90,90,90,90,90,90,90,90,90,90,90,90,90,90,90,90,
  90,90,90,90,90,90,90,90,90,90,90,90,90,90,90,90,90,90,90,90,90,90,90,90,90,90,90,90,90,90,90,90,
  90,90,90,90,90,90,90,90,90,90,90,90,90,90,90,90,90,90,90,90,90,90,90,90,90,90,90,90,90,90,90,90,
  90,90,90,90,90,90,90,90,90,90,90,90,90,90,90,90,90,90,90,90,90,90,90,90,90,90,90,90,90,90,90,90,
  90,90,90,90,90,90,90,90,90,90,90,90,90,90,90,90,90,90,90,90,90,90,90,90,90,90,90,90,90,90,90,90,
  90,90,90,90,90,90,90,90,90,90,90,90,90,90,90,90,90,90,90,90,90,90,90,90,90,90,90,90,90,90,90,90,
  90,90,90,90,90,90,90,90,90,90,90,90,90,90,90,90,90,90,90,90,90,90,90,90,90,90,90,90,90,90,90,90,
  90,90,90,90,90,90,90,90,90,90,90,90,90,90,90,90,90,90,90,90,90,90,90,90,90,90,90,90,90,90,90,90,
  90,90,90,90,90,90,90,90,90,90,90,90,90,90,90,90,90,90,90,90,90,90,90,90,90,90,90,90,90,90,90,90,
  90,90,90,90,90,90,90,90,90,90,90,90,90,90,90,90,90,90,90,90,90,90,90,90,90,90,90,90,90,90,90,90,
  90,90,90,90,90,90,90,90,90,90,90,90,90,90,90,90,90,90,90,90,90,90,90,90,90,90,90,90,90,90,90,90,
  90,90,90,90,90,90,90,90,90,90,90,90,90,90,90,90,90,90,90,90,90,90,90,90,90,90,90,90,90,90,90,90,
  90,90,90,90,90,90,90,90,90,90,90,90,90,90,90,90,0,0,0,0,0,0,0,0,0,0,0,0,0,0,0,0,
  0,0,0,0,0,0,0,0,0,0,0,0,0,0,0,0,0,0,0,0,0,0,0,0,0,0,0,0,0,0,0,0,
  0,0,0,0,0,0,0,0,0,0,0,0,0,0,0,0,240,0,0,0,0,0,0,0,0,0,0,0,0,0,0,0,
  0,0,0,0,0,0,0,0,90,90,90,90,90,90,90,90,90,90,90,90,90,90,90,90,90,90,90,90,90,90,90,90,
  90,90,90,90,90,90,90,90,90,90,90,90,90,90,90,90,90,90,90,90,90,90,90,90,90,90,90,90,90,90,90,90,
  90,90,90,90,90,90,90,90,90,90,90,90,90,90,90,90,90,90,90,90,90,90,90,90,90,90,90,90,90,90,90,90,
  90,90,90,90,90,90,90,90,90,90,90,90,90,90,90,90,90,90,90,90,90,90,90,90,90,90,90,90,90,90,90,90,
  90,90,90,90,90,90,90,90,90,90,90,90,90,90,90,90,90,90,90,90,90,90,90,90,90,90,90,90,90,90,90,90,
  90,90,90,90,90,90,90,90,90,90,90,90,90,90,90,90,90,90,90,90,90,90,90,90,90,90,90,90,90,90,90,90,
  90,90,90,90,90,90,90,90,90,90,90,90,90,90,90,90,90,90,90,90,90,90,90,90,90,90,90,90,90,90,90,90,
  90,90,90,90,90,90,90,90,90,90,90,90,90,90,90,90,90,90,90,90,90,90,90,90,90,90,90,90,90,90,90,90,
  90,90,90,90,90,90,90,90,90,90,90,90,90,90,90,90,90,90,90,90,90,90,90,90,90,90,90,90,90,90,90,90,
  90,90,90,90,90,90,90,90,90,90,90,90,90,90,90,90,90,90,90,90,90,90,90,90,90,90,90,90,90,90,90,90,
  90,90,90,90,90,90,90,90,90,90,90,90,90,90,90,90,90,90,90,90,90,90,90,90,90,90,90,90,90,90,90,90,
  90,90,90,90,90,90,90,90,90,90,90,90,90,90,90,90,90,90,90,90,90,90,90,90,90,90,90,90,90,90,90,90,
  90,90,90,90,90,90,90,90,90,90,90,90,90,90,90,90,90,90,90,90,90,90,90,90,90,90,90,90,90,90,90,90,
  90,90,90,90,90,90,90,90,90,90,90,90,90,90,90,90,90,90,90,90,90,90,90,90,90,90,90,90,90,90,90,90,
  90,90,90,90,90,90,90,90,90,90,90,90,90,90,90,90,90,90,90,90,90,90,90,90,90,90,90,90,90,90,90,90,
  90,90,90,90,90,90,90,90,90,90,90,90,90,90,90,90,90,90,90,90,90,90,90,90,90,90,90,90,90,90,90,90,
  90,90,90,90,90,90,90,90,90,90,90,90,90,90,90,90,90,90,90,90,90,90,90,90,90,90,90,90,90,90,90,90,
  90,90,90,90,90,90,90,90,90,90,90,90,90,90,90,90,90,90,90,90,90,90,90,90,90,90,90,90,90,90,90,90,
  90,90,90,90,90,90,90,90,90,90,90,90,90,90,90,90,90,90,90,90,90,90,90,90,90,90,90,90,90,90,90,90,
  90,90,90,90,90,90,90,90,90,90,90,90,90,90,90,90,90,90,90,90,90,90,90,90,90,90,90,90,90,90,90,90,
  90,90,90,90,90,90,90,90,90,90,90,90,90,90,90,90,90,90,90,90,90,90,90,90,90,90,90,90,90,90,90,90,
  90,90,90,90,90,90,90,90,90,90,90,90,90,90,90,90,90,90,90,90,90,90,90,90,90,90,90,90,90,90,90,90,
  90,90,90,90,90,90,90,90,90,90,90,90,90,90,90,90,90,90,90,90,90,90,90,90,90,90,90,90,90,90,90,90,
  90,90,90,90,90,90,90,90,90,90,90,90,90,90,90,90,90,90,90,90,90,90,90,90,90,90,90,90,90,90,90,90,
  90,90,90,90,90,90,90,90,90,90,90,90,90,90,90,90,90,90,90,90,90,90,90,90,90,90,90,90,90,90,90,90,
  90,90,90,90,90,90,90,90,90,90,90,90,90,90,90,90,0,0,0,0,0,0,0,0,0,0,0,0,0,0,0,0,
  0,0,0,0,0,0,0,0,0,0,0,0,0,0,0,0,16,0,0,0,8,0,0,0,0,0,0,0,0,0,0,0,
  0,0,0,0,0,0,0,0,8,0,0,0,8,0,0,0,0,0,0,0,0,1,1,0,1,1,1,0,2,1,1,0,
  3,1,1,0,4,1,1,0,0,0,0,0,0,0,0,0,0,0,0,0,0,0,0,0,0,0,0,0,0,0,0,0,
  0,0,0,0,0,0,0,0,0,0,0,0,0,0,0,0,0,0,0,0,0,0,0,0,0,0,0,0,0,0,0,0,
  0,0,0,0,0,0,0,0,0,0,0,0,0,0,0,0,0,0,0,0,0,0,0,0,0,0,0,0,0,0,0,0,
  0,0,0,0,0,0,0,0,0,0,0,0,0,0,0,0,0,0,0,0,0,0,0,0,0,0,0,0,0,0,0,0,
  0,0,0,0,0,0,0,0,0,0,0,0,0,0,0,0,0,0,0,0,0,0,0,0,0,0,0,0,0,0,0,0,
// ... 174 lines not shown
  0,0,0,0,0,0,0,0,0,0,0,0,0,0,0,0,0,0,0,0,0,0,0,0,0,0,0,0,0,0,0,0,
  0,0,0,0,0,0,0,0,0,0,0,0,0,0,0,0,0,0,0,0,0,0,0,0,0,0,0,0,0,0,0,0,
  0,0,0,0,0,0,0,0,0,0,0,0,0,0,0,0,0,0,0,0,0,0,0,0,0,0,0,0,0,0,0,0,
  0,0,0,0,0,0,0,0,0,0,0,0,0,0,0,0,0,0,0,0,0,0,0,0,0,0,0,0,0,0,0,0,
  0,0,0,0,0,0,0,0,0,0,0,0,0,0,0,0,0,0,0,0,0,0,0,0,0,0,0,0,0,0,0,0,
  0,0,0,0,0,0,0,0,0,0,0,0,0,0,0,0,0,0,0,0,0,0,0,0,0,0,0,0,0,0,0,0,
  0,0,0,0,0,0,0,0,0,0,0,0,0,0,0,0,0,0,0,0,0,0,0,0,0,0,0,0,0,0,0,0,
  0,0,0,0,0,0,0,0,0,0,0,0,0,0,0,0,0,0,0,0,0,0,0,0,0,0,0,0,0,0,0,0,
  0,0,0,0,0,0,0,0,0,0,0,0,0,0,0,0,0,0,0,0,0,0,0,0,0,0,0,0,0,0,0,0,
  0,0,0,0,0,0,0,0,0,0,0,0,0,0,0,0,0,0,0,0,0,0,0,0,0,0,0,0,0,0,0,0,
  0,0,0,0,0,0,0,0,0,0,0,0,0,0,0,0,0,0,0,0,0,0,0,0,0,0,0,0,0,0,0,0,
  0,0,0,0,0,0,0,0,0,0,0,0,0,0,0,0,0,0,0,0,0,0,0,0,0,0,0,0,0,0,0,0,
  0,0,0,0,0,0,0,0,0,0,0,0,0,0,0,0,0,0,0,0,0,0,0,0,0,0,0,0,90,90,90,90,
  90,90,90,90,0,0,0,0,1,0,0,0,0,0,0,0,90,90,90,90,90,90,90,90,90,90,90,90,90,90,90,90,
  90,90,90,90,90,90,90,90,90,90,90,90,90,90,90,90,90,90,90,90,0,0,0,0,0,0,0,0,0,0,0,0,
  90,90,90,90,90,90,90,90,0,0,0,0,0,0,0,0,90,90,90,90,90,90,90,90,90,90,90,90,90,90,90,90,
  90,90,90,90,90,90,90,90,90,90,90,90,90,90,90,90,0,0,0,0,0,0,0,0,0,0,0,0,0,0,0,0,
  0,0,0,0,0,0,0,0,0,0,0,0,0,0,0,0,0,0,0,0,0,0,0,0,0,0,0,0,0,0,0,0,
  0,0,0,0,0,0,0,0,0,0,0,0,0,0,0,0,0,0,0,0,0,0,0,0,0,0,0,0,0,0,0,0,
  0,0,0,0,0,0,0,0,0,0,0,0,0,0,0,0,0,0,0,0,0,0,0,0,0,0,0,0,0,0,0,0,
  0,0,0,0,0,0,0,0,0,0,0,0,0,0,0,0,0,0,0,0,0,0,0,0,0,0,0,0,0,0,0,0,
  0,0,0,0,0,0,0,0,0,0,0,0,0,0,0,0,0,0,0,0,4,0,0,0,25,0,0,0,25,0,0,0,
  113,2,0,0,11,0,0,0,7,0,0,0,20,0,0,0,6,0,0,0,11,0,0,0,7,0,0,0,11,0,0,0,
  11,0,0,0,1,0,0,0,1,0,0,0,1,0,0,0,1,0,0,0,0,0,0,0,1,0,0,0,6,0,0,0,
  0,0,0,0,1,0,0,0,2,0,0,0,3,0,0,0,4,0,0,0,5,0,0,0,0,0,0,0,0,0,0,0,
  0,0,0,0,0,0,0,0,0,0,0,0,0,0,0,0,0,0,0,0,0,0,0,0,0,0,0,0,0,0,0,0,
  1,0,0,0,11,0,0,0,11,0,0,0,11,0,0,0,11,0,0,0,4,0,0,0,0,0,0,0,0,0,0,0,
  0,0,0,0,0,0,0,0,0,0,0,0,0,0,0,0,0,0,0,0,0,0,0,0,0,0,0,0,0,0,0,0,
  1,0,0,0,2,0,0,0,13,0,0,0,24,0,0,0,35,0,0,0,46,0,0,0,0,0,0,0,0,0,0,0,
  0,0,0,0,0,0,0,0,0,0,0,0,0,0,0,0,0,0,0,0,0,0,0,0,0,0,0,0,0,0,0,0,
  50,0,0,0,7,0,0,0,21,0,0,0,148,0,0,0,21,0,0,0,1,0,0,0,7,0,0,0,136,0,0,0,
  86,0,0,0,6,0,0,0,0,0,0,0,2,0,0,0,114,0,0,0,115,0,0,0,130,0,0,0,131,0,0,0,
  0,0,0,0,68,0,0,0,82,0,0,0,83,0,0,0,0,0,0,0,3,0,0,0,0,0,0,0,50,0,0,0,
  154,0,0,0,144,27,0,0,0,0,0,0,176,10,0,0,192,10,0,0,208,10,0,0,240,10,0,0,200,9,0,0,
  232,9,0,0,8,10,0,0,40,10,0,0,72,10,0,0,104,10,0,0,136,10,0,0,208,13,0,0,216,13,0,0,
  224,13,0,0,128,14,0,0,32,15,0,0,64,15,0,0,152,15,0,0,16,11,0,0,88,16,0,0,96,16,0,0,
  240,15,0,0,16,16,0,0,48,16,0,0,80,16,0,0,124,16,0,0,128,16,0,0,132,16,0,0,156,16,0,0,
  172,16,0,0,0,0,0,0,0,0,0,0,0,0,0,0,192,16,0,0,184,16,0,0,188,16,0,0,176,16,0,0,
  92,16,0,0,140,16,0,0,128,26,0,0,144,26,0,0,136,16,0,0,0,0,0,0,0,0,0,0,0,0,0,0,
  0,0,0,0,0,0,0,0,0,0,0,0,0,0,0,0,0,0,0,0,0,0,0,0,0,0,0,0,0,0,0,0,
  0,0,0,0,0,0,0,0,0,0,0,0,0,0,0,0,0,0,0,0,0,0,0,0,0,0,0,0,0,0,0,0,
  0,0,0,0,0,0,0,0,0,0,0,0,0,0,0,0,0,0,0,0,0,0,0,0,0,0,0,0,0,0,0,0,
  0,0,0,0,0,0,0,0,0,0,0,0,0,0,0,0,0,0,0,0,0,0,0,0,174,158,29,2,117,209,69,23,
  82,184,30,5,226,225,225,1,117,209,69,23,187,232,162,11,18,17,17,17,140,219,104,0,164,112,61,10,187,232,162,11,
  13,195,48,12,0,0,0,0,0,0,0,0,0,0,0,0,90,90,90,90,90,90,90,90,90,90,90,90,90,90,90,90,
  90,90,90,90,90,90,90,90,90,90,90,90,90,90,90,90,90,90,90,90,90,90,90,90,90,90,90,90,90,90,90,90,
  90,90,90,90,90,90,90,90,90,90,90,90,90,90,90,90,90,90,90,90,90,90,90,90,90,90,90,90,90,90,90,90,
  90,90,90,90,90,90,90,90,90,90,90,90,90,90,90,90,90,90,90,90,90,90,90,90,90,90,90,90,90,90,90,90,
  90,90,90,90,90,90,90,90,90,90,90,90,90,90,90,90,90,90,90,90,90,90,90,90,90,90,90,90,90,90,90,90,
  90,90,90,90,90,90,90,90,90,90,90,90,90,90,90,90,90,90,90,90,90,90,90,90,90,90,90,90,90,90,90,90,
  90,90,90,90,90,90,90,90,90,90,90,90,90,90,90,90,90,90,90,90,90,90,90,90,90,90,90,90,90,90,90,90,
  90,90,90,90,90,90,90,90,90,90,90,90,90,90,90,90,90,90,90,90,90,90,90,90,90,90,90,90,90,90,90,90,
  90,90,90,90,90,90,90,90,90,90,90,90,90,90,90,90,90,90,90,90,90,90,90,90,90,90,90,90,90,90,90,90,
  90,90,90,90,90,90,90,90,90,90,90,90,90,90,90,90,90,90,90,90,90,90,90,90,90,90,90,90,90,90,90,90,
  90,90,90,90,90,90,90,90,90,90,90,90,90,90,90,90,90,90,90,90,90,90,90,90,90,90,90,90,90,90,90,90,
  90,90,90,90,90,90,90,90,90,90,90,90,90,90,90,90,90,90,90,90,90,90,90,90,90,90,90,90,90,90,90,90,
  90,90,90,90,90,90,90,90,90,90,90,90,90,90,90,90,90,90,90,90,90,90,90,90,90,90,90,90,90,90,90,90,
  90,90,90,90,90,90,90,90,90,90,90,90,90,90,90,90,90,90,90,90,90,90,90,90,90,90,90,90,90,90,90,90,
  90,90,90,90,90,90,90,90,90,90,90,90,90,90,90,90,90,90,90,90,90,90,90,90,90,90,90,90,90,90,90,90,
  90,90,90,90,90,90,90,90,90,90,90,90,90,90,90,90,90,90,90,90,90,90,90,90,90,90,90,90,90,90,90,90,
  90,90,90,90,90,90,90,90,90,90,90,90,90,90,90,90,90,90,90,90,90,90,90,90,90,90,90,90,90,90,90,90,
  90,90,90,90,90,90,90,90,90,90,90,90,90,90,90,90,90,90,90,90,90,90,90,90,90,90,90,90,90,90,90,90,
  90,90,90,90,90,90,90,90,90,90,90,90,90,90,90,90,90,90,90,90,90,90,90,90,90,90,90,90,90,90,90,90,
  90,90,90,90,90,90,90,90,90,90,90,90,90,90,90,90,90,90,90,90,90,90,90,90,90,90,90,90,90,90,90,90,
  90,90,90,90,90,90,90,90,90,90,90,90,90,90,90,90,90,90,90,90,90,90,90,90,90,90,90,90,90,90,90,90,
  90,90,90,90,90,90,90,90,90,90,90,90,90,90,90,90,90,90,90,90,90,90,90,90,90,90,90,90,90,90,90,90,
  90,90,90,90,90,90,90,90,90,90,90,90,90,90,90,90,90,90,90,90,90,90,90,90,90,90,90,90,90,90,90,90,
  90,90,90,90,90,90,90,90,90,90,90,90,90,90,90,90,90,90,90,90,90,90,90,90,90,90,90,90,90,90,90,90,
  90,90,90,90,90,90,90,90,90,90,90,90,90,90,90,90,90,90,90,90,90,90,90,90,90,90,90,90,90,90,90,90,
  90,90,90,90,90,90,90,90,90,90,90,90,90,90,90,90,0,0,0,0,0,0,0,0,0,0,0,0,0,0,0,0,
  0,0,0,0,0,0,0,0,0,0,0,0,0,0,0,0,0,0,0,0,0,0,0,0,0,0,0,0,0,0,0,0,
  0,0,0,0,0,0,0,0,0,0,0,0,0,0,0,0,128,2,0,0,0,0,0,0,0,0,0,0,0,0,0,0,
  0,0,0,0,0,0,0,0,90,90,90,90,90,90,90,90,90,90,90,90,90,90,90,90,90,90,90,90,90,90,90,90,
  90,90,90,90,90,90,90,90,90,90,90,90,90,90,90,90,90,90,90,90,90,90,90,90,90,90,90,90,90,90,90,90,
  90,90,90,90,90,90,90,90,90,90,90,90,90,90,90,90,90,90,90,90,90,90,90,90,90,90,90,90,90,90,90,90,
  90,90,90,90,90,90,90,90,90,90,90,90,90,90,90,90,90,90,90,90,90,90,90,90,90,90,90,90,90,90,90,90,
  90,90,90,90,90,90,90,90,90,90,90,90,90,90,90,90,90,90,90,90,90,90,90,90,90,90,90,90,90,90,90,90,
  90,90,90,90,90,90,90,90,90,90,90,90,90,90,90,90,90,90,90,90,90,90,90,90,90,90,90,90,90,90,90,90,
  90,90,90,90,90,90,90,90,90,90,90,90,90,90,90,90,90,90,90,90,90,90,90,90,90,90,90,90,90,90,90,90,
  90,90,90,90,90,90,90,90,90,90,90,90,90,90,90,90,90,90,90,90,90,90,90,90,90,90,90,90,90,90,90,90,
  90,90,90,90,90,90,90,90,90,90,90,90,90,90,90,90,90,90,90,90,90,90,90,90,90,90,90,90,90,90,90,90,
  90,90,90,90,90,90,90,90,90,90,90,90,90,90,90,90,90,90,90,90,90,90,90,90,90,90,90,90,90,90,90,90,
  90,90,90,90,90,90,90,90,90,90,90,90,90,90,90,90,90,90,90,90,90,90,90,90,90,90,90,90,90,90,90,90,
  90,90,90,90,90,90,90,90,90,90,90,90,90,90,90,90,90,90,90,90,90,90,90,90,90,90,90,90,90,90,90,90,
  90,90,90,90,90,90,90,90,90,90,90,90,90,90,90,90,90,90,90,90,90,90,90,90,90,90,90,90,90,90,90,90,
  90,90,90,90,90,90,90,90,90,90,90,90,90,90,90,90,90,90,90,90,90,90,90,90,90,90,90,90,90,90,90,90,
  90,90,90,90,90,90,90,90,90,90,90,90,90,90,90,90,90,90,90,90,90,90,90,90,90,90,90,90,90,90,90,90,
  90,90,90,90,90,90,90,90,90,90,90,90,90,90,90,90,90,90,90,90,90,90,90,90,90,90,90,90,90,90,90,90,
  90,90,90,90,90,90,90,90,90,90,90,90,90,90,90,90,90,90,90,90,90,90,90,90,90,90,90,90,90,90,90,90,
  90,90,90,90,90,90,90,90,90,90,90,90,90,90,90,90,90,90,90,90,90,90,90,90,90,90,90,90,90,90,90,90,
  90,90,90,90,90,90,90,90,90,90,90,90,90,90,90,90,90,90,90,90,90,90,90,90,90,90,90,90,90,90,90,90,
  90,90,90,90,90,90,90,90,90,90,90,90,90,90,90,90,90,90,90,90,90,90,90,90,90,90,90,90,90,90,90,90,
  90,90,90,90,90,90,90,90,90,90,90,90,90,90,90,90,90,90,90,90,90,90,90,90,90,90,90,90,90,90,90,90,
  90,90,90,90,90,90,90,90,90,90,90,90,90,90,90,90,90,90,90,90,90,90,90,90,90,90,90,90,90,90,90,90,
  90,90,90,90,90,90,90,90,90,90,90,90,90,90,90,90,90,90,90,90,90,90,90,90,90,90,90,90,90,90,90,90,
  90,90,90,90,90,90,90,90,90,90,90,90,90,90,90,90,90,90,90,90,90,90,90,90,90,90,90,90,90,90,90,90,
  90,90,90,90,90,90,90,90,90,90,90,90,90,90,90,90,90,90,90,90,90,90,90,90,90,90,90,90,90,90,90,90,
  90,90,90,90,90,90,90,90,90,90,90,90,90,90,90,90,0,0,0,0,0,0,0,0,0,0,0,0,0,0,0,0,
  0,0,0,0,0,0,0,0,0,0,0,0,0,0,0,0,32,1,0,0,128,0,0,0,0,0,0,0,56,0,0,0,
  88,0,0,0,120,0,0,0,0,1,0,0,28,1,0,0,0,0,0,0,0,1,1,0,8,255,1,0,8,255,2,0,
  8,255,3,0,8,255,4,0,8,255,5,0,8,255,6,0,8,255,7,0,8,255,8,0,8,255,9,0,8,255,10,0,
  8,255,11,0,5,1,1,0,5,1,1,0,5,1,1,0,5,1,1,0,5,1,1,0,5,1,1,0,5,1,1,0,
  5,1,1,0,5,1,1,0,5,1,1,0,5,1,1,0,16,255,1,0,16,255,2,0,16,255,3,0,16,255,4,0,
  16,255,5,0,16,255,6,0,16,255,7,0,16,255,8,0,16,255,9,0,16,255,10,0,16,255,11,0,6,1,1,0,
  6,1,1,0,6,1,1,0,6,1,1,0,6,1,1,0,6,1,1,0,6,1,1,0,6,1,1,0,6,1,1,0,
// ... 174 lines not shown
  0,0,0,0,0,0,0,0,0,0,0,0,0,0,0,0,0,0,0,0,0,0,0,0,0,0,0,0,0,0,0,0,
  0,0,0,0,0,0,0,0,0,0,0,0,0,0,0,0,0,0,0,0,0,0,0,0,0,0,0,0,0,0,0,0,
  0,0,0,0,0,0,0,0,0,0,0,0,0,0,0,0,0,0,0,0,0,0,0,0,0,0,0,0,0,0,0,0,
  0,0,0,0,0,0,0,0,0,0,0,0,0,0,0,0,0,0,0,0,0,0,0,0,0,0,0,0,0,0,0,0,
  0,0,0,0,0,0,0,0,0,0,0,0,0,0,0,0,0,0,0,0,0,0,0,0,0,0,0,0,0,0,0,0,
  0,0,0,0,0,0,0,0,0,0,0,0,0,0,0,0,0,0,0,0,0,0,0,0,0,0,0,0,0,0,0,0,
  0,0,0,0,0,0,0,0,0,0,0,0,0,0,0,0,0,0,0,0,0,0,0,0,0,0,0,0,0,0,0,0,
  0,0,0,0,0,0,0,0,0,0,0,0,0,0,0,0,0,0,0,0,0,0,0,0,0,0,0,0,0,0,0,0,
  0,0,0,0,0,0,0,0,0,0,0,0,0,0,0,0,0,0,0,0,0,0,0,0,0,0,0,0,0,0,0,0,
  0,0,0,0,0,0,0,0,0,0,0,0,0,0,0,0,0,0,0,0,0,0,0,0,0,0,0,0,0,0,0,0,
  0,0,0,0,0,0,0,0,0,0,0,0,0,0,0,0,0,0,0,0,0,0,0,0,0,0,0,0,0,0,0,0,
  0,0,0,0,0,0,0,0,0,0,0,0,0,0,0,0,0,0,0,0,0,0,0,0,0,0,0,0,0,0,0,0,
  0,0,0,0,0,0,0,0,0,0,0,0,0,0,0,0,0,0,0,0,0,0,0,0,0,0,0,0,90,90,90,90,
  90,90,90,90,0,0,0,0,1,0,0,0,0,0,0,0,90,90,90,90,90,90,90,90,90,90,90,90,90,90,90,90,
  90,90,90,90,90,90,90,90,90,90,90,90,90,90,90,90,90,90,90,90,0,0,0,0,0,0,0,0,0,0,0,0,
  90,90,90,90,90,90,90,90,0,0,0,0,0,0,0,0,90,90,90,90,90,90,90,90,90,90,90,90,90,90,90,90,
  90,90,90,90,90,90,90,90,90,90,90,90,90,90,90,90,0,0,0,0,0,0,0,0,0,0,0,0,0,0,0,0,
  0,0,0,0,0,0,0,0,0,0,0,0,0,0,0,0,0,0,0,0,0,0,0,0,0,0,0,0,0,0,0,0,
  0,0,0,0,0,0,0,0,0,0,0,0,0,0,0,0,0,0,0,0,0,0,0,0,0,0,0,0,0,0,0,0,
  0,0,0,0,0,0,0,0,0,0,0,0,0,0,0,0,0,0,0,0,0,0,0,0,0,0,0,0,0,0,0,0,
  0,0,0,0,0,0,0,0,0,0,0,0,0,0,0,0,0,0,0,0,0,0,0,0,0,0,0,0,0,0,0,0,
  0,0,0,0,0,0,0,0,0,0,0,0,0,0,0,0,0,0,0,0,4,0,0,0,25,0,0,0,25,0,0,0,
  113,2,0,0,11,0,0,0,7,0,0,0,20,0,0,0,6,0,0,0,11,0,0,0,7,0,0,0,11,0,0,0,
  11,0,0,0,1,0,0,0,1,0,0,0,1,0,0,0,1,0,0,0,0,0,0,0,0,0,0,0,6,0,0,0,
  0,0,0,0,1,0,0,0,2,0,0,0,3,0,0,0,4,0,0,0,5,0,0,0,0,0,0,0,0,0,0,0,
  0,0,0,0,0,0,0,0,0,0,0,0,0,0,0,0,0,0,0,0,0,0,0,0,0,0,0,0,0,0,0,0,
  1,0,0,0,11,0,0,0,11,0,0,0,11,0,0,0,11,0,0,0,4,0,0,0,0,0,0,0,0,0,0,0,
  0,0,0,0,0,0,0,0,0,0,0,0,0,0,0,0,0,0,0,0,0,0,0,0,0,0,0,0,0,0,0,0,
  1,0,0,0,2,0,0,0,13,0,0,0,24,0,0,0,35,0,0,0,46,0,0,0,0,0,0,0,0,0,0,0,
  0,0,0,0,0,0,0,0,0,0,0,0,0,0,0,0,0,0,0,0,0,0,0,0,0,0,0,0,0,0,0,0,
  50,0,0,0,0,0,0,0,0,0,0,0,1,0,0,0,0,0,0,0,1,0,0,0,1,0,0,0,136,0,0,0,
  86,0,0,0,6,0,0,0,0,0,0,0,2,0,0,0,114,0,0,0,115,0,0,0,130,0,0,0,131,0,0,0,
  0,0,0,0,68,0,0,0,82,0,0,0,83,0,0,0,0,0,0,0,3,0,0,0,0,0,0,0,50,0,0,0,
  1,0,0,0,144,27,0,0,0,0,0,0,176,10,0,0,192,10,0,0,208,10,0,0,240,10,0,0,200,9,0,0,
  232,9,0,0,8,10,0,0,40,10,0,0,72,10,0,0,104,10,0,0,136,10,0,0,208,13,0,0,216,13,0,0,
  224,13,0,0,128,14,0,0,32,15,0,0,64,15,0,0,152,15,0,0,16,11,0,0,88,16,0,0,96,16,0,0,
  240,15,0,0,16,16,0,0,48,16,0,0,80,16,0,0,124,16,0,0,128,16,0,0,132,16,0,0,156,16,0,0,
  172,16,0,0,0,0,0,0,0,0,0,0,0,0,0,0,192,16,0,0,184,16,0,0,188,16,0,0,176,16,0,0,
  92,16,0,0,140,16,0,0,128,26,0,0,144,26,0,0,136,16,0,0,0,0,0,0,0,0,0,0,0,0,0,0,
  0,0,0,0,0,0,0,0,0,0,0,0,0,0,0,0,0,0,0,0,0,0,0,0,0,0,0,0,0,0,0,0,
  0,0,0,0,0,0,0,0,0,0,0,0,0,0,0,0,0,0,0,0,0,0,0,0,0,0,0,0,0,0,0,0,
  0,0,0,0,0,0,0,0,0,0,0,0,0,0,0,0,0,0,0,0,0,0,0,0,0,0,0,0,0,0,0,0,
  0,0,0,0,0,0,0,0,0,0,0,0,0,0,0,0,0,0,0,0,0,0,0,0,174,158,29,2,117,209,69,23,
  82,184,30,5,226,225,225,1,117,209,69,23,187,232,162,11,18,17,17,17,140,219,104,0,164,112,61,10,0,0,0,0,
  0,0,0,0,0,0,0,0,0,0,0,0,0,0,0,0,90,90,90,90,90,90,90,90,90,90,90,90,90,90,90,90,
  90,90,90,90,90,90,90,90,90,90,90,90,90,90,90,90,90,90,90,90,90,90,90,90,90,90,90,90,90,90,90,90,
  90,90,90,90,90,90,90,90,90,90,90,90,90,90,90,90,90,90,90,90,90,90,90,90,90,90,90,90,90,90,90,90,
  90,90,90,90,90,90,90,90,90,90,90,90,90,90,90,90,90,90,90,90,90,90,90,90,90,90,90,90,90,90,90,90,
  90,90,90,90,90,90,90,90,90,90,90,90,90,90,90,90,90,90,90,90,90,90,90,90,90,90,90,90,90,90,90,90,
  90,90,90,90,90,90,90,90,90,90,90,90,90,90,90,90,90,90,90,90,90,90,90,90,90,90,90,90,90,90,90,90,
  90,90,90,90,90,90,90,90,90,90,90,90,90,90,90,90,90,90,90,90,90,90,90,90,90,90,90,90,90,90,90,90,
  90,90,90,90,90,90,90,90,90,90,90,90,90,90,90,90,90,90,90,90,90,90,90,90,90,90,90,90,90,90,90,90,
  90,90,90,90,90,90,90,90,90,90,90,90,90,90,90,90,90,90,90,90,90,90,90,90,90,90,90,90,90,90,90,90,
  90,90,90,90,90,90,90,90,90,90,90,90,90,90,90,90,90,90,90,90,90,90,90,90,90,90,90,90,90,90,90,90,
  90,90,90,90,90,90,90,90,90,90,90,90,90,90,90,90,90,90,90,90,90,90,90,90,90,90,90,90,90,90,90,90,
  90,90,90,90,90,90,90,90,90,90,90,90,90,90,90,90,90,90,90,90,90,90,90,90,90,90,90,90,90,90,90,90,
  90,90,90,90,90,90,90,90,90,90,90,90,90,90,90,90,90,90,90,90,90,90,90,90,90,90,90,90,90,90,90,90,
  90,90,90,90,90,90,90,90,90,90,90,90,90,90,90,90,90,90,90,90,90,90,90,90,90,90,90,90,90,90,90,90,
  90,90,90,90,90,90,90,90,90,90,90,90,90,90,90,90,90,90,90,90,90,90,90,90,90,90,90,90,90,90,90,90,
  90,90,90,90,90,90,90,90,90,90,90,90,90,90,90,90,90,90,90,90,90,90,90,90,90,90,90,90,90,90,90,90,
  90,90,90,90,90,90,90,90,90,90,90,90,90,90,90,90,90,90,90,90,90,90,90,90,90,90,90,90,90,90,90,90,
  90,90,90,90,90,90,90,90,90,90,90,90,90,90,90,90,90,90,90,90,90,90,90,90,90,90,90,90,90,90,90,90,
  90,90,90,90,90,90,90,90,90,90,90,90,90,90,90,90,90,90,90,90,90,90,90,90,90,90,90,90,90,90,90,90,
  90,90,90,90,90,90,90,90,90,90,90,90,90,90,90,90,90,90,90,90,90,90,90,90,90,90,90,90,90,90,90,90,
  90,90,90,90,90,90,90,90,90,90,90,90,90,90,90,90,90,90,90,90,90,90,90,90,90,90,90,90,90,90,90,90,
  90,90,90,90,90,90,90,90,90,90,90,90,90,90,90,90,90,90,90,90,90,90,90,90,90,90,90,90,90,90,90,90,
  90,90,90,90,90,90,90,90,90,90,90,90,90,90,90,90,90,90,90,90,90,90,90,90,90,90,90,90,90,90,90,90,
  90,90,90,90,90,90,90,90,90,90,90,90,90,90,90,90,90,90,90,90,90,90,90,90,90,90,90,90,90,90,90,90,
  90,90,90,90,90,90,90,90,90,90,90,90,90,90,90,90,90,90,90,90,90,90,90,90,90,90,90,90,90,90,90,90,
  90,90,90,90,90,90,90,90,90,90,90,90,90,90,90,90,0,0,0,0,0,0,0,0,0,0,0,0,0,0,0,0,
  0,0,0,0,0,0,0,0,0,0,0,0,0,0,0,0,0,0,0,0,0,0,0,0,0,0,0,0,0,0,0,0,
  0,0,0,0,0,0,0,0,0,0,0,0,0,0,0,0,128,2,0,0,0,0,0,0,0,0,0,0,0,0,0,0,
  0,0,0,0,0,0,0,0,90,90,90,90,90,90,90,90,90,90,90,90,90,90,90,90,90,90,90,90,90,90,90,90,
  90,90,90,90,90,90,90,90,90,90,90,90,90,90,90,90,90,90,90,90,90,90,90,90,90,90,90,90,90,90,90,90,
  90,90,90,90,90,90,90,90,90,90,90,90,90,90,90,90,90,90,90,90,90,90,90,90,90,90,90,90,90,90,90,90,
  90,90,90,90,90,90,90,90,90,90,90,90,90,90,90,90,90,90,90,90,90,90,90,90,90,90,90,90,90,90,90,90,
  90,90,90,90,90,90,90,90,90,90,90,90,90,90,90,90,90,90,90,90,90,90,90,90,90,90,90,90,90,90,90,90,
  90,90,90,90,90,90,90,90,90,90,90,90,90,90,90,90,90,90,90,90,90,90,90,90,90,90,90,90,90,90,90,90,
  90,90,90,90,90,90,90,90,90,90,90,90,90,90,90,90,90,90,90,90,90,90,90,90,90,90,90,90,90,90,90,90,
  90,90,90,90,90,90,90,90,90,90,90,90,90,90,90,90,90,90,90,90,90,90,90,90,90,90,90,90,90,90,90,90,
  90,90,90,90,90,90,90,90,90,90,90,90,90,90,90,90,90,90,90,90,90,90,90,90,90,90,90,90,90,90,90,90,
  90,90,90,90,90,90,90,90,90,90,90,90,90,90,90,90,90,90,90,90,90,90,90,90,90,90,90,90,90,90,90,90,
  90,90,90,90,90,90,90,90,90,90,90,90,90,90,90,90,90,90,90,90,90,90,90,90,90,90,90,90,90,90,90,90,
  90,90,90,90,90,90,90,90,90,90,90,90,90,90,90,90,90,90,90,90,90,90,90,90,90,90,90,90,90,90,90,90,
  90,90,90,90,90,90,90,90,90,90,90,90,90,90,90,90,90,90,90,90,90,90,90,90,90,90,90,90,90,90,90,90,
  90,90,90,90,90,90,90,90,90,90,90,90,90,90,90,90,90,90,90,90,90,90,90,90,90,90,90,90,90,90,90,90,
  90,90,90,90,90,90,90,90,90,90,90,90,90,90,90,90,90,90,90,90,90,90,90,90,90,90,90,90,90,90,90,90,
  90,90,90,90,90,90,90,90,90,90,90,90,90,90,90,90,90,90,90,90,90,90,90,90,90,90,90,90,90,90,90,90,
  90,90,90,90,90,90,90,90,90,90,90,90,90,90,90,90,90,90,90,90,90,90,90,90,90,90,90,90,90,90,90,90,
  90,90,90,90,90,90,90,90,90,90,90,90,90,90,90,90,90,90,90,90,90,90,90,90,90,90,90,90,90,90,90,90,
  90,90,90,90,90,90,90,90,90,90,90,90,90,90,90,90,90,90,90,90,90,90,90,90,90,90,90,90,90,90,90,90,
  90,90,90,90,90,90,90,90,90,90,90,90,90,90,90,90,90,90,90,90,90,90,90,90,90,90,90,90,90,90,90,90,
  90,90,90,90,90,90,90,90,90,90,90,90,90,90,90,90,90,90,90,90,90,90,90,90,90,90,90,90,90,90,90,90,
  90,90,90,90,90,90,90,90,90,90,90,90,90,90,90,90,90,90,90,90,90,90,90,90,90,90,90,90,90,90,90,90,
  90,90,90,90,90,90,90,90,90,90,90,90,90,90,90,90,90,90,90,90,90,90,90,90,90,90,90,90,90,90,90,90,
  90,90,90,90,90,90,90,90,90,90,90,90,90,90,90,90,90,90,90,90,90,90,90,90,90,90,90,90,90,90,90,90,
  90,90,90,90,90,90,90,90,90,90,90,90,90,90,90,90,90,90,90,90,90,90,90,90,90,90,90,90,90,90,90,90,
  90,90,90,90,90,90,90,90,90,90,90,90,90,90,90,90,0,0,0,0,0,0,0,0,0,0,0,0,0,0,0,0,
  0,0,0,0,0,0,0,0,0,0,0,0,0,0,0,0,32,1,0,0,128,0,0,0,0,0,0,0,56,0,0,0,
  88,0,0,0,120,0,0,0,0,1,0,0,28,1,0,0,0,0,0,0,0,1,1,0,8,255,1,0,8,255,2,0,
  8,255,3,0,8,255,4,0,8,255,5,0,8,255,6,0,8,255,7,0,8,255,8,0,8,255,9,0,8,255,10,0,
  8,255,11,0,5,1,1,0,5,1,1,0,5,1,1,0,5,1,1,0,5,1,1,0,5,1,1,0,5,1,1,0,
  5,1,1,0,5,1,1,0,5,1,1,0,5,1,1,0,16,255,1,0,16,255,2,0,16,255,3,0,16,255,4,0,
  16,255,5,0,16,255,6,0,16,255,7,0,16,255,8,0,16,255,9,0,16,255,10,0,16,255,11,0,6,1,1,0,
  6,1,1,0,6,1,1,0,6,1,1,0,6,1,1,0,6,1,1,0,6,1,1,0,6,1,1,0,6,1,1,0,
// ... 174 lines not shown
  0,0,0,0,0,0,0,0,0,0,0,0,0,0,0,0,0,0,0,0,0,0,0,0,0,0,0,0,0,0,0,0,
  0,0,0,0,0,0,0,0,0,0,0,0,0,0,0,0,0,0,0,0,0,0,0,0,0,0,0,0,0,0,0,0,
  0,0,0,0,0,0,0,0,0,0,0,0,0,0,0,0,0,0,0,0,0,0,0,0,0,0,0,0,0,0,0,0,
  0,0,0,0,0,0,0,0,0,0,0,0,0,0,0,0,0,0,0,0,0,0,0,0,0,0,0,0,0,0,0,0,
  0,0,0,0,0,0,0,0,0,0,0,0,0,0,0,0,0,0,0,0,0,0,0,0,0,0,0,0,0,0,0,0,
  0,0,0,0,0,0,0,0,0,0,0,0,0,0,0,0,0,0,0,0,0,0,0,0,0,0,0,0,0,0,0,0,
  0,0,0,0,0,0,0,0,0,0,0,0,0,0,0,0,0,0,0,0,0,0,0,0,0,0,0,0,0,0,0,0,
  0,0,0,0,0,0,0,0,0,0,0,0,0,0,0,0,0,0,0,0,0,0,0,0,0,0,0,0,0,0,0,0,
  0,0,0,0,0,0,0,0,0,0,0,0,0,0,0,0,0,0,0,0,0,0,0,0,0,0,0,0,0,0,0,0,
  0,0,0,0,0,0,0,0,0,0,0,0,0,0,0,0,0,0,0,0,0,0,0,0,0,0,0,0,0,0,0,0,
  0,0,0,0,0,0,0,0,0,0,0,0,0,0,0,0,0,0,0,0,0,0,0,0,0,0,0,0,0,0,0,0,
  0,0,0,0,0,0,0,0,0,0,0,0,0,0,0,0,0,0,0,0,0,0,0,0,0,0,0,0,0,0,0,0,
  0,0,0,0,0,0,0,0,0,0,0,0,0,0,0,0,0,0,0,0,0,0,0,0,0,0,0,0,90,90,90,90,
  90,90,90,90,1,0,0,0,0,0,0,0,0,0,0,0,90,90,90,90,90,90,90,90,90,90,90,90,90,90,90,90,
  90,90,90,90,90,90,90,90,90,90,90,90,90,90,90,90,90,90,90,90,0,0,0,0,0,0,0,0,0,0,0,0,
  90,90,90,90,90,90,90,90,0,0,0,0,0,0,0,0,90,90,90,90,90,90,90,90,90,90,90,90,90,90,90,90,
  90,90,90,90,90,90,90,90,90,90,90,90,90,90,90,90,0,0,0,0,0,0,0,0,0,0,0,0,0,0,0,0,
  0,0,0,0,0,0,0,0,0,0,0,0,0,0,0,0,0,0,0,0,0,0,0,0,0,0,0,0,0,0,0,0,
  0,0,0,0,0,0,0,0,0,0,0,0,0,0,0,0,0,0,0,0,0,0,0,0,0,0,0,0,0,0,0,0,
  0,0,0,0,0,0,0,0,0,0,0,0,0,0,0,0,0,0,0,0,0,0,0,0,0,0,0,0,0,0,0,0,
  0,0,0,0,0,0,0,0,0,0,0,0,0,0,0,0,0,0,0,0,0,0,0,0,0,0,0,0,0,0,0,0,
  0,0,0,0,0,0,0,0,0,0,0,0,0,0,0,0,0,0,0,0,4,0,0,0,25,0,0,0,25,0,0,0,
  113,2,0,0,11,0,0,0,7,0,0,0,20,0,0,0,6,0,0,0,11,0,0,0,7,0,0,0,11,0,0,0,
  11,0,0,0,1,0,0,0,1,0,0,0,1,0,0,0,1,0,0,0,0,0,0,0,1,0,0,0,6,0,0,0,
  0,0,0,0,1,0,0,0,2,0,0,0,3,0,0,0,4,0,0,0,5,0,0,0,0,0,0,0,0,0,0,0,
  0,0,0,0,0,0,0,0,0,0,0,0,0,0,0,0,0,0,0,0,0,0,0,0,0,0,0,0,0,0,0,0,
  1,0,0,0,11,0,0,0,11,0,0,0,11,0,0,0,11,0,0,0,4,0,0,0,0,0,0,0,0,0,0,0,
  0,0,0,0,0,0,0,0,0,0,0,0,0,0,0,0,0,0,0,0,0,0,0,0,0,0,0,0,0,0,0,0,
  1,0,0,0,2,0,0,0,13,0,0,0,24,0,0,0,35,0,0,0,46,0,0,0,0,0,0,0,0,0,0,0,
  0,0,0,0,0,0,0,0,0,0,0,0,0,0,0,0,0,0,0,0,0,0,0,0,0,0,0,0,0,0,0,0,
  50,0,0,0,7,0,0,0,21,0,0,0,148,0,0,0,21,0,0,0,1,0,0,0,7,0,0,0,136,0,0,0,
  86,0,0,0,8,0,0,0,0,0,0,0,2,0,0,0,114,0,0,0,115,0,0,0,130,0,0,0,131,0,0,0,
  0,0,0,0,68,0,0,0,82,0,0,0,83,0,0,0,0,0,0,0,3,0,0,0,0,0,0,0,50,0,0,0,
  154,0,0,0,208,16,0,0,0,0,0,0,176,10,0,0,192,10,0,0,208,10,0,0,240,10,0,0,200,9,0,0,
  232,9,0,0,8,10,0,0,40,10,0,0,72,10,0,0,104,10,0,0,136,10,0,0,208,13,0,0,216,13,0,0,
  224,13,0,0,128,14,0,0,32,15,0,0,64,15,0,0,152,15,0,0,16,11,0,0,88,16,0,0,96,16,0,0,
  240,15,0,0,16,16,0,0,48,16,0,0,80,16,0,0,124,16,0,0,128,16,0,0,132,16,0,0,156,16,0,0,
  172,16,0,0,0,0,0,0,0,0,0,0,0,0,0,0,192,16,0,0,184,16,0,0,188,16,0,0,176,16,0,0,
  92,16,0,0,140,16,0,0,0,0,0,0,0,0,0,0,136,16,0,0,0,0,0,0,0,0,0,0,0,0,0,0,
  0,0,0,0,0,0,0,0,0,0,0,0,0,0,0,0,0,0,0,0,0,0,0,0,0,0,0,0,0,0,0,0,
  0,0,0,0,0,0,0,0,0,0,0,0,0,0,0,0,0,0,0,0,0,0,0,0,0,0,0,0,0,0,0,0,
  0,0,0,0,0,0,0,0,0,0,0,0,0,0,0,0,0,0,0,0,0,0,0,0,0,0,0,0,0,0,0,0,
  0,0,0,0,0,0,0,0,0,0,0,0,0,0,0,0,0,0,0,0,0,0,0,0,174,158,29,2,117,209,69,23,
  82,184,30,5,226,225,225,1,117,209,69,23,187,232,162,11,18,17,17,17,140,219,104,0,164,112,61,10,187,232,162,11,
  13,195,48,12,0,0,0,0,0,0,0,0,0,0,0,0,90,90,90,90,90,90,90,90,90,90,90,90,90,90,90,90,
  90,90,90,90,90,90,90,90,90,90,90,90,90,90,90,90,90,90,90,90,90,90,90,90,90,90,90,90,90,90,90,90,
  90,90,90,90,90,90,90,90,90,90,90,90,90,90,90,90,90,90,90,90,90,90,90,90,90,90,90,90,90,90,90,90,
  90,90,90,90,90,90,90,90,90,90,90,90,90,90,90,90,90,90,90,90,90,90,90,90,90,90,90,90,90,90,90,90,
  90,90,90,90,90,90,90,90,90,90,90,90,90,90,90,90,90,90,90,90,90,90,90,90,90,90,90,90,90,90,90,90,
  90,90,90,90,90,90,90,90,90,90,90,90,90,90,90,90,90,90,90,90,90,90,90,90,90,90,90,90,90,90,90,90,
  90,90,90,90,90,90,90,90,90,90,90,90,90,90,90,90,90,90,90,90,90,90,90,90,90,90,90,90,90,90,90,90,
  90,90,90,90,90,90,90,90,90,90,90,90,90,90,90,90,90,90,90,90,90,90,90,90,90,90,90,90,90,90,90,90,
  90,90,90,90,90,90,90,90,90,90,90,90,90,90,90,90,90,90,90,90,90,90,90,90,90,90,90,90,90,90,90,90,
  90,90,90,90,90,90,90,90,90,90,90,90,90,90,90,90,90,90,90,90,90,90,90,90,90,90,90,90,90,90,90,90,
  90,90,90,90,90,90,90,90,90,90,90,90,90,90,90,90,90,90,90,90,90,90,90,90,90,90,90,90,90,90,90,90,
  90,90,90,90,90,90,90,90,90,90,90,90,90,90,90,90,90,90,90,90,90,90,90,90,90,90,90,90,90,90,90,90,
  90,90,90,90,90,90,90,90,90,90,90,90,90,90,90,90,90,90,90,90,90,90,90,90,90,90,90,90,90,90,90,90,
  90,90,90,90,90,90,90,90,90,90,90,90,90,90,90,90,90,90,90,90,90,90,90,90,90,90,90,90,90,90,90,90,
  90,90,90,90,90,90,90,90,90,90,90,90,90,90,90,90,90,90,90,90,90,90,90,90,90,90,90,90,90,90,90,90,
  90,90,90,90,90,90,90,90,90,90,90,90,90,90,90,90,90,90,90,90,90,90,90,90,90,90,90,90,90,90,90,90,
  90,90,90,90,90,90,90,90,90,90,90,90,90,90,90,90,90,90,90,90,90,90,90,90,90,90,90,90,90,90,90,90,
  90,90,90,90,90,90,90,90,90,90,90,90,90,90,90,90,90,90,90,90,90,90,90,90,90,90,90,90,90,90,90,90,
  90,90,90,90,90,90,90,90,90,90,90,90,90,90,90,90,90,90,90,90,90,90,90,90,90,90,90,90,90,90,90,90,
  90,90,90,90,90,90,90,90,90,90,90,90,90,90,90,90,90,90,90,90,90,90,90,90,90,90,90,90,90,90,90,90,
  90,90,90,90,90,90,90,90,90,90,90,90,90,90,90,90,90,90,90,90,90,90,90,90,90,90,90,90,90,90,90,90,
  90,90,90,90,90,90,90,90,90,90,90,90,90,90,90,90,90,90,90,90,90,90,90,90,90,90,90,90,90,90,90,90,
  90,90,90,90,90,90,90,90,90,90,90,90,90,90,90,90,90,90,90,90,90,90,90,90,90,90,90,90,90,90,90,90,
  90,90,90,90,90,90,90,90,90,90,90,90,90,90,90,90,90,90,90,90,90,90,90,90,90,90,90,90,90,90,90,90,
  90,90,90,90,90,90,90,90,90,90,90,90,90,90,90,90,90,90,90,90,90,90,90,90,90,90,90,90,90,90,90,90,
  90,90,90,90,90,90,90,90,90,90,90,90,90,90,90,90,0,0,0,0,0,0,0,0,0,0,0,0,0,0,0,0,
  0,0,0,0,0,0,0,0,0,0,0,0,0,0,0,0,0,0,0,0,0,0,0,0,0,0,0,0,0,0,0,0,
  0,0,0,0,0,0,0,0,0,0,0,0,0,0,0,0,128,2,0,0,0,0,0,0,0,0,0,0,0,0,0,0,
  0,0,0,0,0,0,0,0,90,90,90,90,90,90,90,90,90,90,90,90,90,90,90,90,90,90,90,90,90,90,90,90,
  90,90,90,90,90,90,90,90,90,90,90,90,90,90,90,90,90,90,90,90,90,90,90,90,90,90,90,90,90,90,90,90,
  90,90,90,90,90,90,90,90,90,90,90,90,90,90,90,90,90,90,90,90,90,90,90,90,90,90,90,90,90,90,90,90,
  90,90,90,90,90,90,90,90,90,90,90,90,90,90,90,90,90,90,90,90,90,90,90,90,90,90,90,90,90,90,90,90,
  90,90,90,90,90,90,90,90,90,90,90,90,90,90,90,90,90,90,90,90,90,90,90,90,90,90,90,90,90,90,90,90,
  90,90,90,90,90,90,90,90,90,90,90,90,90,90,90,90,90,90,90,90,90,90,90,90,90,90,90,90,90,90,90,90,
  90,90,90,90,90,90,90,90,90,90,90,90,90,90,90,90,90,90,90,90,90,90,90,90,90,90,90,90,90,90,90,90,
  90,90,90,90,90,90,90,90,90,90,90,90,90,90,90,90,90,90,90,90,90,90,90,90,90,90,90,90,90,90,90,90,
  90,90,90,90,90,90,90,90,90,90,90,90,90,90,90,90,90,90,90,90,90,90,90,90,90,90,90,90,90,90,90,90,
  90,90,90,90,90,90,90,90,90,90,90,90,90,90,90,90,90,90,90,90,90,90,90,90,90,90,90,90,90,90,90,90,
  90,90,90,90,90,90,90,90,90,90,90,90,90,90,90,90,90,90,90,90,90,90,90,90,90,90,90,90,90,90,90,90,
  90,90,90,90,90,90,90,90,90,90,90,90,90,90,90,90,90,90,90,90,90,90,90,90,90,90,90,90,90,90,90,90,
  90,90,90,90,90,90,90,90,90,90,90,90,90,90,90,90,90,90,90,90,90,90,90,90,90,90,90,90,90,90,90,90,
  90,90,90,90,90,90,90,90,90,90,90,90,90,90,90,90,90,90,90,90,90,90,90,90,90,90,90,90,90,90,90,90,
  90,90,90,90,90,90,90,90,90,90,90,90,90,90,90,90,90,90,90,90,90,90,90,90,90,90,90,90,90,90,90,90,
  90,90,90,90,90,90,90,90,90,90,90,90,90,90,90,90,90,90,90,90,90,90,90,90,90,90,90,90,90,90,90,90,
  90,90,90,90,90,90,90,90,90,90,90,90,90,90,90,90,90,90,90,90,90,90,90,90,90,90,90,90,90,90,90,90,
  90,90,90,90,90,90,90,90,90,90,90,90,90,90,90,90,90,90,90,90,90,90,90,90,90,90,90,90,90,90,90,90,
  90,90,90,90,90,90,90,90,90,90,90,90,90,90,90,90,90,90,90,90,90,90,90,90,90,90,90,90,90,90,90,90,
  90,90,90,90,90,90,90,90,90,90,90,90,90,90,90,90,90,90,90,90,90,90,90,90,90,90,90,90,90,90,90,90,
  90,90,90,90,90,90,90,90,90,90,90,90,90,90,90,90,90,90,90,90,90,90,90,90,90,90,90,90,90,90,90,90,
  90,90,90,90,90,90,90,90,90,90,90,90,90,90,90,90,90,90,90,90,90,90,90,90,90,90,90,90,90,90,90,90,
  90,90,90,90,90,90,90,90,90,90,90,90,90,90,90,90,90,90,90,90,90,90,90,90,90,90,90,90,90,90,90,90,
  90,90,90,90,90,90,90,90,90,90,90,90,90,90,90,90,90,90,90,90,90,90,90,90,90,90,90,90,90,90,90,90,
  90,90,90,90,90,90,90,90,90,90,90,90,90,90,90,90,90,90,90,90,90,90,90,90,90,90,90,90,90,90,90,90,
  90,90,90,90,90,90,90,90,90,90,90,90,90,90,90,90,0,0,0,0,0,0,0,0,0,0,0,0,0,0,0,0,
  0,0,0,0,0,0,0,0,0,0,0,0,0,0,0,0,32,1,0,0,128,0,0,0,0,0,0,0,56,0,0,0,
  88,0,0,0,120,0,0,0,0,1,0,0,28,1,0,0,0,0,0,0,0,1,1,0,8,255,1,0,8,255,2,0,
  8,255,3,0,8,255,4,0,8,255,5,0,8,255,6,0,8,255,7,0,8,255,8,0,8,255,9,0,8,255,10,0,
  8,255,11,0,5,1,1,0,5,1,1,0,5,1,1,0,5,1,1,0,5,1,1,0,5,1,1,0,5,1,1,0,
  5,1,1,0,5,1,1,0,5,1,1,0,5,1,1,0,16,255,1,0,16,255,2,0,16,255,3,0,16,255,4,0,
  16,255,5,0,16,255,6,0,16,255,7,0,16,255,8,0,16,255,9,0,16,255,10,0,16,255,11,0,6,1,1,0,
  6,1,1,0,6,1,1,0,6,1,1,0,6,1,1,0,6,1,1,0,6,1,1,0,6,1,1,0,6,1,1,0,
// ... 453 lines not shown
  0,0,0,0,0,0,0,0,0,0,0,0,0,0,0,0,0,0,0,0,0,0,0,0,0,0,0,0,0,0,0,0,
  0,0,0,0,0,0,0,0,0,0,0,0,0,0,0,0,0,0,0,0,0,0,0,0,0,0,0,0,0,0,0,0,
  0,0,0,0,0,0,0,0,0,0,0,0,0,0,0,0,0,0,0,0,0,0,0,0,0,0,0,0,0,0,0,0,
  0,0,0,0,0,0,0,0,0,0,0,0,0,0,0,0,0,0,0,0,0,0,0,0,0,0,0,0,0,0,0,0,
  0,0,0,0,0,0,0,0,0,0,0,0,0,0,0,0,0,0,0,0,0,0,0,0,0,0,0,0,0,0,0,0,
  0,0,0,0,0,0,0,0,0,0,0,0,0,0,0,0,0,0,0,0,0,0,0,0,0,0,0,0,0,0,0,0,
  0,0,0,0,0,0,0,0,0,0,0,0,0,0,0,0,0,0,0,0,0,0,0,0,0,0,0,0,0,0,0,0,
  0,0,0,0,0,0,0,0,0,0,0,0,0,0,0,0,0,0,0,0,0,0,0,0,0,0,0,0,0,0,0,0,
  0,0,0,0,0,0,0,0,0,0,0,0,0,0,0,0,0,0,0,0,0,0,0,0,0,0,0,0,0,0,0,0,
  0,0,0,0,0,0,0,0,0,0,0,0,0,0,0,0,0,0,0,0,0,0,0,0,0,0,0,0,0,0,0,0,
  0,0,0,0,0,0,0,0,0,0,0,0,0,0,0,0,0,0,0,0,0,0,0,0,0,0,0,0,0,0,0,0,
  0,0,0,0,0,0,0,0,0,0,0,0,0,0,0,0,0,0,0,0,0,0,0,0,0,0,0,0,0,0,0,0,
  0,0,0,0,0,0,0,0,0,0,0,0,0,0,0,0,0,0,0,0,0,0,0,0,0,0,0,0,90,90,90,90,
  90,90,90,90,1,0,0,0,0,0,0,0,0,0,0,0,90,90,90,90,90,90,90,90,90,90,90,90,90,90,90,90,
  90,90,90,90,90,90,90,90,90,90,90,90,90,90,90,90,90,90,90,90,0,0,0,0,0,0,0,0,0,0,0,0,
  90,90,90,90,90,90,90,90,1,0,0,0,0,0,0,0,90,90,90,90,90,90,90,90,90,90,90,90,90,90,90,90,
  90,90,90,90,90,90,90,90,90,90,90,90,90,90,90,90,0,0,0,0,0,0,0,0,0,0,0,0,0,0,0,0,
  0,0,0,0,0,0,0,0,0,0,0,0,0,0,0,0,0,0,0,0,0,0,0,0,0,0,0,0,0,0,0,0,
  0,0,0,0,0,0,0,0,0,0,0,0,0,0,0,0,0,0,0,0,0,0,0,0,0,0,0,0,0,0,0,0,
  0,0,0,0,0,0,0,0,0,0,0,0,0,0,0,0,0,0,0,0,0,0,0,0,0,0,0,0,0,0,0,0,
  0,0,0,0,0,0,0,0,0,0,0,0,0,0,0,0,0,0,0,0,0,0,0,0,0,0,0,0,0,0,0,0,
  0,0,0,0,0,0,0,0,0,0,0,0,0,0,0,0,0,0,0,0,4,0,0,0,15,0,0,0,15,0,0,0,
  225,0,0,0,0,0,0,0,0,0,0,0,0,0,0,0,5,0,0,0,11,0,0,0,6,0,0,0,11,0,0,0,
  11,0,0,0,1,0,0,0,0,0,0,0,1,0,0,0,0,0,0,0,0,0,0,0,0,0,0,0,2,0,0,0,
  0,0,0,0,5,0,0,0,0,0,0,0,0,0,0,0,0,0,0,0,0,0,0,0,0,0,0,0,0,0,0,0,
  0,0,0,0,0,0,0,0,0,0,0,0,0,0,0,0,0,0,0,0,0,0,0,0,0,0,0,0,0,0,0,0,
  1,0,0,0,4,0,0,0,0,0,0,0,0,0,0,0,0,0,0,0,0,0,0,0,0,0,0,0,0,0,0,0,
  0,0,0,0,0,0,0,0,0,0,0,0,0,0,0,0,0,0,0,0,0,0,0,0,0,0,0,0,0,0,0,0,
  1,0,0,0,2,0,0,0,0,0,0,0,0,0,0,0,0,0,0,0,0,0,0,0,0,0,0,0,0,0,0,0,
  0,0,0,0,0,0,0,0,0,0,0,0,0,0,0,0,0,0,0,0,0,0,0,0,0,0,0,0,0,0,0,0,
  6,0,0,0,0,0,0,0,0,0,0,0,1,0,0,0,0,0,0,0,1,0,0,0,1,0,0,0,9,0,0,0,
  4,0,0,0,5,0,0,0,0,0,0,0,2,0,0,0,2,0,0,0,3,0,0,0,3,0,0,0,4,0,0,0,
  0,0,0,0,0,0,0,0,0,0,0,0,1,0,0,0,0,0,0,0,0,0,0,0,0,0,0,0,6,0,0,0,
  1,0,0,0,64,6,0,0,0,0,0,0,112,4,0,0,128,4,0,0,144,4,0,0,176,4,0,0,136,3,0,0,
  168,3,0,0,200,3,0,0,232,3,0,0,8,4,0,0,40,4,0,0,72,4,0,0,0,0,0,0,0,0,0,0,
  0,0,0,0,0,0,0,0,0,0,0,0,0,0,0,0,0,0,0,0,0,0,0,0,0,0,0,0,0,0,0,0,
  0,0,0,0,0,0,0,0,0,0,0,0,0,0,0,0,208,4,0,0,212,4,0,0,216,4,0,0,240,4,0,0,
  0,5,0,0,0,0,0,0,0,0,0,0,0,0,0,0,32,5,0,0,16,5,0,0,20,5,0,0,8,5,0,0,
  0,0,0,0,224,4,0,0,48,5,0,0,64,5,0,0,220,4,0,0,0,0,0,0,0,0,0,0,0,0,0,0,
  0,0,0,0,0,0,0,0,0,0,0,0,0,0,0,0,0,0,0,0,0,0,0,0,0,0,0,0,0,0,0,0,
  0,0,0,0,0,0,0,0,0,0,0,0,0,0,0,0,0,0,0,0,0,0,0,0,0,0,0,0,0,0,0,0,
  0,0,0,0,0,0,0,0,0,0,0,0,0,0,0,0,0,0,0,0,0,0,0,0,0,0,0,0,0,0,0,0,
  0,0,0,0,0,0,0,0,0,0,0,0,0,0,0,0,0,0,0,0,0,0,0,0,174,158,29,2,117,209,69,23,
  171,170,170,42,29,199,113,28,0,0,0,0,0,0,0,0,0,0,0,32,104,69,35,1,18,17,17,17,0,0,0,0,
  0,0,0,0,0,0,0,0,0,0,0,0,0,0,0,0,90,90,90,90,90,90,90,90,90,90,90,90,90,90,90,90,
  90,90,90,90,90,90,90,90,90,90,90,90,90,90,90,90,90,90,90,90,90,90,90,90,90,90,90,90,90,90,90,90,
  90,90,90,90,90,90,90,90,90,90,90,90,90,90,90,90,90,90,90,90,90,90,90,90,90,90,90,90,90,90,90,90,
  90,90,90,90,90,90,90,90,90,90,90,90,90,90,90,90,90,90,90,90,90,90,90,90,90,90,90,90,90,90,90,90,
  90,90,90,90,90,90,90,90,90,90,90,90,90,90,90,90,90,90,90,90,90,90,90,90,90,90,90,90,90,90,90,90,
  90,90,90,90,90,90,90,90,90,90,90,90,90,90,90,90,90,90,90,90,90,90,90,90,90,90,90,90,90,90,90,90,
  90,90,90,90,90,90,90,90,90,90,90,90,90,90,90,90,90,90,90,90,90,90,90,90,90,90,90,90,90,90,90,90,
  90,90,90,90,90,90,90,90,90,90,90,90,90,90,90,90,90,90,90,90,90,90,90,90,90,90,90,90,90,90,90,90,
  90,90,90,90,90,90,90,90,90,90,90,90,90,90,90,90,90,90,90,90,90,90,90,90,90,90,90,90,90,90,90,90,
  90,90,90,90,90,90,90,90,90,90,90,90,90,90,90,90,90,90,90,90,90,90,90,90,90,90,90,90,90,90,90,90,
  90,90,90,90,90,90,90,90,90,90,90,90,90,90,90,90,90,90,90,90,90,90,90,90,90,90,90,90,90,90,90,90,
  90,90,90,90,90,90,90,90,90,90,90,90,90,90,90,90,90,90,90,90,90,90,90,90,90,90,90,90,90,90,90,90,
  90,90,90,90,90,90,90,90,90,90,90,90,90,90,90,90,90,90,90,90,90,90,90,90,90,90,90,90,90,90,90,90,
  90,90,90,90,90,90,90,90,90,90,90,90,90,90,90,90,90,90,90,90,90,90,90,90,90,90,90,90,90,90,90,90,
  90,90,90,90,90,90,90,90,90,90,90,90,90,90,90,90,90,90,90,90,90,90,90,90,90,90,90,90,90,90,90,90,
  90,90,90,90,90,90,90,90,90,90,90,90,90,90,90,90,90,90,90,90,90,90,90,90,90,90,90,90,90,90,90,90,
  90,90,90,90,90,90,90,90,90,90,90,90,90,90,90,90,90,90,90,90,90,90,90,90,90,90,90,90,90,90,90,90,
  90,90,90,90,90,90,90,90,90,90,90,90,90,90,90,90,90,90,90,90,90,90,90,90,90,90,90,90,90,90,90,90,
  90,90,90,90,90,90,90,90,90,90,90,90,90,90,90,90,90,90,90,90,90,90,90,90,90,90,90,90,90,90,90,90,
  90,90,90,90,90,90,90,90,90,90,90,90,90,90,90,90,90,90,90,90,90,90,90,90,90,90,90,90,90,90,90,90,
  90,90,90,90,90,90,90,90,90,90,90,90,90,90,90,90,90,90,90,90,90,90,90,90,90,90,90,90,90,90,90,90,
  90,90,90,90,90,90,90,90,90,90,90,90,90,90,90,90,90,90,90,90,90,90,90,90,90,90,90,90,90,90,90,90,
  90,90,90,90,90,90,90,90,90,90,90,90,90,90,90,90,90,90,90,90,90,90,90,90,90,90,90,90,90,90,90,90,
  90,90,90,90,90,90,90,90,90,90,90,90,90,90,90,90,90,90,90,90,90,90,90,90,90,90,90,90,90,90,90,90,
  90,90,90,90,90,90,90,90,90,90,90,90,90,90,90,90,90,90,90,90,90,90,90,90,90,90,90,90,90,90,90,90,
  90,90,90,90,90,90,90,90,90,90,90,90,90,90,90,90,0,0,0,0,0,0,0,0,0,0,0,0,0,0,0,0,
  0,0,0,0,0,0,0,0,0,0,0,0,0,0,0,0,0,0,0,0,0,0,0,0,0,0,0,0,0,0,0,0,
  0,0,0,0,0,0,0,0,0,0,0,0,0,0,0,0,240,0,0,0,0,0,0,0,0,0,0,0,0,0,0,0,
  0,0,0,0,0,0,0,0,90,90,90,90,90,90,90,90,90,90,90,90,90,90,90,90,90,90,90,90,90,90,90,90,
  90,90,90,90,90,90,90,90,90,90,90,90,90,90,90,90,90,90,90,90,90,90,90,90,90,90,90,90,90,90,90,90,
  90,90,90,90,90,90,90,90,90,90,90,90,90,90,90,90,90,90,90,90,90,90,90,90,90,90,90,90,90,90,90,90,
  90,90,90,90,90,90,90,90,90,90,90,90,90,90,90,90,90,90,90,90,90,90,90,90,90,90,90,90,90,90,90,90,
  90,90,90,90,90,90,90,90,90,90,90,90,90,90,90,90,90,90,90,90,90,90,90,90,90,90,90,90,90,90,90,90,
  90,90,90,90,90,90,90,90,90,90,90,90,90,90,90,90,90,90,90,90,90,90,90,90,90,90,90,90,90,90,90,90,
  90,90,90,90,90,90,90,90,90,90,90,90,90,90,90,90,90,90,90,90,90,90,90,90,90,90,90,90,90,90,90,90,
  90,90,90,90,90,90,90,90,90,90,90,90,90,90,90,90,90,90,90,90,90,90,90,90,90,90,90,90,90,90,90,90,
  90,90,90,90,90,90,90,90,90,90,90,90,90,90,90,90,90,90,90,90,90,90,90,90,90,90,90,90,90,90,90,90,
  90,90,90,90,90,90,90,90,90,90,90,90,90,90,90,90,90,90,90,90,90,90,90,90,90,90,90,90,90,90,90,90,
  90,90,90,90,90,90,90,90,90,90,90,90,90,90,90,90,90,90,90,90,90,90,90,90,90,90,90,90,90,90,90,90,
  90,90,90,90,90,90,90,90,90,90,90,90,90,90,90,90,90,90,90,90,90,90,90,90,90,90,90,90,90,90,90,90,
  90,90,90,90,90,90,90,90,90,90,90,90,90,90,90,90,90,90,90,90,90,90,90,90,90,90,90,90,90,90,90,90,
  90,90,90,90,90,90,90,90,90,90,90,90,90,90,90,90,90,90,90,90,90,90,90,90,90,90,90,90,90,90,90,90,
  90,90,90,90,90,90,90,90,90,90,90,90,90,90,90,90,90,90,90,90,90,90,90,90,90,90,90,90,90,90,90,90,
  90,90,90,90,90,90,90,90,90,90,90,90,90,90,90,90,90,90,90,90,90,90,90,90,90,90,90,90,90,90,90,90,
  90,90,90,90,90,90,90,90,90,90,90,90,90,90,90,90,90,90,90,90,90,90,90,90,90,90,90,90,90,90,90,90,
  90,90,90,90,90,90,90,90,90,90,90,90,90,90,90,90,90,90,90,90,90,90,90,90,90,90,90,90,90,90,90,90,
  90,90,90,90,90,90,90,90,90,90,90,90,90,90,90,90,90,90,90,90,90,90,90,90,90,90,90,90,90,90,90,90,
  90,90,90,90,90,90,90,90,90,90,90,90,90,90,90,90,90,90,90,90,90,90,90,90,90,90,90,90,90,90,90,90,
  90,90,90,90,90,90,90,90,90,90,90,90,90,90,90,90,90,90,90,90,90,90,90,90,90,90,90,90,90,90,90,90,
  90,90,90,90,90,90,90,90,90,90,90,90,90,90,90,90,90,90,90,90,90,90,90,90,90,90,90,90,90,90,90,90,
  90,90,90,90,90,90,90,90,90,90,90,90,90,90,90,90,90,90,90,90,90,90,90,90,90,90,90,90,90,90,90,90,
  90,90,90,90,90,90,90,90,90,90,90,90,90,90,90,90,90,90,90,90,90,90,90,90,90,90,90,90,90,90,90,90,
  90,90,90,90,90,90,90,90,90,90,90,90,90,90,90,90,90,90,90,90,90,90,90,90,90,90,90,90,90,90,90,90,
  90,90,90,90,90,90,90,90,90,90,90,90,90,90,90,90,0,0,0,0,0,0,0,0,0,0,0,0,0,0,0,0,
  0,0,0,0,0,0,0,0,0,0,0,0,0,0,0,0,16,0,0,0,8,0,0,0,0,0,0,0,0,0,0,0,
  0,0,0,0,0,0,0,0,8,0,0,0,8,0,0,0,0,0,0,0,0,1,1,0,1,1,1,0,2,1,1,0,
  3,1,1,0,4,1,1,0,0,0,0,0,0,0,0,0,0,0,0,0,0,0,0,0,0,0,0,0,0,0,0,0,
  0,0,0,0,0,0,0,0,0,0,0,0,0,0,0,0,0,0,0,0,0,0,0,0,0,0,0,0,0,0,0,0,
  0,0,0,0,0,0,0,0,0,0,0,0,0,0,0,0,0,0,0,0,0,0,0,0,0,0,0,0,0,0,0,0,
  0,0,0,0,0,0,0,0,0,0,0,0,0,0,0,0,0,0,0,0,0,0,0,0,0,0,0,0,0,0,0,0,
  0,0,0,0,0,0,0,0,0,0,0,0,0,0,0,0,0,0,0,0,0,0,0,0,0,0,0,0,0,0,0,0,
// ... 83 lines not shown
```

Measured before the change: 779.0 million agent-steps/s.

## Add packed 8-bit cell plane to shrink per-step cell loads

After: 790.4 million agent-steps/s (median of 6 runs). 1.01x the previous value.

```diff
diff --git a/ai-economist_amd/csrc/aie_capi.hip b/ai-economist_amd/csrc/aie_capi.hip
--- a/ai-economist_amd/csrc/aie_capi.hip
+++ b/ai-economist_amd/csrc/aie_capi.hip
@@ -129,6 +129,10 @@
   uint32_t* w = reinterpret_cast<uint32_t*>(arena + P.a_records + (int64_t)e * P.rec_bytes + P.o_cells) + cell;
   const uint32_t fl = flags[shared ? cell : q];
   *w = (*w & 0x00ffffffu) | (fl << 24);
+  if (P.o_cells8) {
+    uint8_t* b = arena + P.a_records + (int64_t)e * P.rec_bytes + P.o_cells8 + cell;
+    *b = (uint8_t)((*b & ~7u) | (fl & 7u));
+  }
 }
 
 __global__ void __launch_bounds__(64) aie_src_list_kernel(const aie_params* __restrict__ params, uint8_t* __restrict__ arena) {
diff --git a/ai-economist_amd/csrc/aie_gtb_state.h b/ai-economist_amd/csrc/aie_gtb_state.h
--- a/ai-economist_amd/csrc/aie_gtb_state.h
+++ b/ai-economist_amd/csrc/aie_gtb_state.h
@@ -177,6 +177,61 @@
 __device__ __forceinline__ void dirty_agent_moved(MTL& m, int i) {
   if (i < 32) m.mv0 |= 1u << i; else m.mv1 |= 1u << (i - 32);
 }
+__device__ __forceinline__ uint4 cells8_expand(uint32_t d) {
+  const uint32_t st = (d >> 3) & 0x01010101u, wd = (d >> 4) & 0x01010101u, fl = d & 0x07070707u;
+  const uint32_t ow = ((((d >> 5) & 0x07070707u) | 0x80808080u) - 0x01010101u) ^ 0x80808080u;
+  const uint32_t sw01 = __builtin_amdgcn_perm(wd, st, 0x05010400u), sw23 = __builtin_amdgcn_perm(wd, st, 0x07030602u);
+  const uint32_t of01 = __builtin_amdgcn_perm(fl, ow, 0x05010400u), of23 = __builtin_amdgcn_perm(fl, ow, 0x07030602u);
+  uint4 w;
+  w.x = __builtin_amdgcn_perm(of01, sw01, 0x05040100u);
+  w.y = __builtin_amdgcn_perm(of01, sw01, 0x07060302u);
+  w.z = __builtin_amdgcn_perm(of23, sw23, 0x05040100u);
+  w.w = __builtin_amdgcn_perm(of23, sw23, 0x07060302u);
+  return w;
+}
+__device__ __forceinline__ void load_record_step(const Ctx& c, const uint8_t* __restrict__ arena, int wave, int nwaves) {
+  if (!c.P.o_cells8) {
+    MT none;
+    load_record(c, arena, none, wave, nwaves, -1);
+    return;
+  }
+  const uint8_t* g = arena + (int64_t)c.e * c.P.rec_bytes;
+  const uint4* src = reinterpret_cast<const uint4*>(g);
+  const uint32_t* plane = reinterpret_cast<const uint32_t*>(g + c.P.o_cells8);
+  uint4* dst = reinterpret_cast<uint4*>(c.rec);
+  const int nq = rec_lds_bytes(c.P) >> 4, q0 = (4 * c.P.HW) >> 4;
+  const int q = q0 + wave * AIE_NT + c.tid, k0 = wave == 0 ? c.tid : q0;
+  const bool hu = q < nq, h0 = k0 < q0, h1 = k0 + AIE_NT < q0, h2 = k0 + 2 * AIE_NT < q0;
+  uint4 u = {0u, 0u, 0u, 0u};
+  uint32_t d0 = 0u, d1 = 0u, d2 = 0u;
+  if (hu) u = src[q];
+  if (h0) d0 = plane[k0];
+  if (h1) d1 = plane[k0 + AIE_NT];
+  if (h2) d2 = plane[k0 + 2 * AIE_NT];
+  if (hu) dst[q] = u;
+  if (h0) dst[k0] = cells8_expand(d0);
+  if (h1) dst[k0 + AIE_NT] = cells8_expand(d1);
+  if (h2) dst[k0 + 2 * AIE_NT] = cells8_expand(d2);
+  for (int qq = q + nwaves * AIE_NT; qq < nq; qq += nwaves * AIE_NT) dst[qq] = src[qq];
+  for (int k = k0 + 3 * AIE_NT; k < q0; k += AIE_NT) dst[k] = cells8_expand(plane[k]);
+}
+__device__ __forceinline__ void load_record_cells(const Ctx& c, const uint8_t* __restrict__ arena, int wave, int nwaves) {
+  const uint4* src = reinterpret_cast<const uint4*>(arena + (int64_t)c.e * c.P.rec_bytes);
+  uint4* dst = reinterpret_cast<uint4*>(c.rec);
+  const int q0 = (4 * c.P.HW) >> 4;
+  for (int q = wave * AIE_NT + c.tid; q < q0; q += nwaves * AIE_NT) dst[q] = src[q];
+}
+__device__ __forceinline__ void store_cells8(const Ctx& c, uint8_t* __restrict__ arena, int wave = 0, int nwaves = 1) {
+  uint32_t* plane = reinterpret_cast<uint32_t*>(arena + (int64_t)c.e * c.P.rec_bytes + c.P.o_cells8);
+  const int nd = ((c.P.HW + 15) >> 4) << 2;
+  for (int k = wave * AIE_NT + c.tid; k < nd; k += nwaves * AIE_NT) {
+    uint32_t d = 0;
+#pragma unroll
+    for (int j = 0; j < 4; ++j)
+      if (4 * k + j < c.P.HW) d |= aie_cell_pack8(R_CELLS(c)[4 * k + j]) << (8 * j);
+    plane[k] = d;
+  }
+}
 __device__ __forceinline__ void store_record_step(const Ctx& c, uint8_t* __restrict__ arena, int wave, int nwaves) {
   uint8_t* g = arena + (int64_t)c.e * c.P.rec_bytes;
   uint4* dst = reinterpret_cast<uint4*>(g);
@@ -187,8 +242,11 @@
   for (int q = q0 + wave * AIE_NT + c.tid; q < nq; q += nwaves * AIE_NT) dst[q] = src[q];
   if (wave == nwaves - 1 && q0 > 0 && c.tid < cnt) {
     const int cell = (int)dirty_list(c)[c.tid];
-    reinterpret_cast<uint32_t*>(g + c.P.o_cells)[cell] = R_CELLS(c)[cell];
-  }
-}
-
-}
+    const uint32_t w = R_CELLS(c)[cell];
+    reinterpret_cast<uint32_t*>(g + c.P.o_cells)[cell] = w;
+    if (c.P.o_cells8) (g + c.P.o_cells8)[cell] = (uint8_t)aie_cell_pack8(w);
+  }
+  if (c.P.o_cells8 && q0 == 0) store_cells8(c, arena, wave, nwaves);
+}
+
+}
diff --git a/ai-economist_amd/csrc/aie_kernels.hip b/ai-economist_amd/csrc/aie_kernels.hip
--- a/ai-economist_amd/csrc/aie_kernels.hip
+++ b/ai-economist_amd/csrc/aie_kernels.hip
@@ -83,11 +83,15 @@
     else A.act = 0;
     if (TRACE && R.dev_trace && c.tid == 0) R.dev_trace[12 * blockIdx.x] = wall_clock64();
     if (TRACE && R.dev_trace && c.tid == 0) R.dev_trace[12 * blockIdx.x + 9] = wall_clock64();
-    MT none;
-    load_record(c, arena, none, 0, 2, -1);
-    __syncthreads();
+    load_record_step(c, arena, 0, 2);
+    __syncthreads();
+    const bool cells_stale = P.o_cells8 != 0 && uni(*R_I32(c, o_obs_valid)) == 0;
+    if (cells_stale) {
+      load_record_cells(c, arena, 0, 2);
+      __syncthreads();
+    }
     if (TRACE && R.dev_trace && c.tid == 0) R.dev_trace[12 * blockIdx.x + 8] = wall_clock64();
-    MTL ml{draw_w, 0, 0u, -AIE_MT_N, 0, 0u, 0u, 0, 0, 0, FAST ? reinterpret_cast<uint32_t*>(c.rec + P.o_mt) : gkey, draw_cap, FAST};
+    MTL ml{draw_w, 0, 0u, -AIE_MT_N, cells_stale ? AIE_DIRTY_CAP + 1 : 0, 0u, 0u, 0, 0, 0, FAST ? reinterpret_cast<uint32_t*>(c.rec + P.o_mt) : gkey, draw_cap, FAST};
     ml.pos = ml.base = uni(*R_I32(c, o_mt_pos));
     ml.avail = ml.cap < AIE_MT_N - ml.pos ? ml.cap : AIE_MT_N - ml.pos;
     if (FAST) {
@@ -163,7 +167,7 @@
     MT m;
     mt_init(m, P);
     const int gpos = *reinterpret_cast<const int32_t*>(grec + P.o_mt_pos);
-    load_record(c, arena, m, 1, 2, -1);
+    load_record_step(c, arena, 1, 2);
     if (skip & AIE_DEV_SKIP_DRAW_WINDOW) {}
     else if (FAST) draw_window_publish_fast(draw_w, draw_cap, (uint32_t)uni((int)gkey[0]), (uint32_t)uni((int)gkey[1]), (uint32_t)uni((int)gkey[2]), uni(gpos), c.tid);
     else draw_window_publish_from_hbm(draw_w, draw_cap, gkey, uni(gpos), c.tid);
@@ -174,6 +178,10 @@
       for (int q = c.tid; q < P.MA; q += AIE_NT) const_cast<uint32_t*>(c.mtab)[q] = P.mask_test[q];
     }
     __syncthreads();
+    if (P.o_cells8 != 0 && uni(*R_I32(c, o_obs_valid)) == 0) {
+      load_record_cells(c, arena, 1, 2);
+      __syncthreads();
+    }
     if (!(skip & AIE_DEV_SKIP_LOCMAP)) rebuild_locmap(c);
     __syncthreads();
     SrcList src;
@@ -509,6 +517,7 @@
   }
   __syncthreads();
   store_record(c, arena, m);
+  if (P.o_cells8) store_cells8(c, arena);
 }
 }
 
diff --git a/ai-economist_amd/csrc/aie_layout.h b/ai-economist_amd/csrc/aie_layout.h
--- a/ai-economist_amd/csrc/aie_layout.h
+++ b/ai-economist_amd/csrc/aie_layout.h
@@ -133,7 +133,8 @@
   int32_t saez_global_cap, saez_pad_;
   int64_t a_layout_prob;
   int64_t a_layout_stage, a_layout_tag, a_layout_ctl;
-  int32_t layout_stage_stride, layout_pad_;
+  int32_t layout_stage_stride;
+  int32_t o_cells8;
   int64_t a_src_list;
   int32_t o_tax_saez_rates;
   int32_t o_tax_saez_obs_rates;
@@ -303,6 +304,9 @@
 static inline int aie__record_src_list(const aie_config* c) {
   return c->scenario == AIE_SCN_GTB && !(aie__shared_src_list(c) && c->rng_mode == AIE_RNG_FAST);
 }
+static inline int aie__cell_plane(const aie_config* c) {
+  return c->scenario == AIE_SCN_GTB && c->max_health[0] == 1 && c->max_health[1] == 1 && c->n_agents <= 7;
+}
 static inline int32_t aie__rng_state_words(const aie_config* c) { return c->rng_mode == AIE_RNG_FAST ? 4 : AIE_MT_N; }
 AIE_HD static inline int aie__layout_staged(const aie_config* c) {
   return c->scenario == AIE_SCN_GTB && c->layout_gen != AIE_LAYOUT_FIXED && c->rng_mode == AIE_RNG_FAST;
@@ -374,6 +378,13 @@
 #define AIE_CELL_PACK(st, wd, own, fl) \
   ((uint32_t)(st) | ((uint32_t)(wd) << 8) | (((uint32_t)(own) & 0xffu) << 16) | ((uint32_t)(fl) << 24))
 
+AIE_HD static inline uint32_t aie_cell_pack8(uint32_t w) {
+  return (AIE_CELL_FLAGS(w) & 7u) | ((w & 1u) << 3) | (((w >> 8) & 1u) << 4) | (((((w >> 16) & 0xffu) + 1u) & 7u) << 5);
+}
+AIE_HD static inline uint32_t aie_cell_unpack8(uint32_t b) {
+  return AIE_CELL_PACK((b >> 3) & 1u, (b >> 4) & 1u, (b >> 5) - 1u, b & 7u);
+}
+
 #define AIE_ORD_AGENT(o) ((o) & 0xff)
 #define AIE_ORD_PRICE(o) (((o) >> 8) & 0xff)
 #define AIE_ORD_LIFE(o) (((o) >> 16) & 0xffff)
diff --git a/ai-economist_amd/csrc/aie_layout_build.h b/ai-economist_amd/csrc/aie_layout_build.h
--- a/ai-economist_amd/csrc/aie_layout_build.h
+++ b/ai-economist_amd/csrc/aie_layout_build.h
@@ -818,6 +818,7 @@
     p->o_src_n = aie__rec(&cur, 16, 16);
     p->o_src_list = aie__rec(&cur, 2 * AIE_SRC_CAP, 16);
   }
+  p->o_cells8 = aie__cell_plane(c) ? aie__rec(&cur, (int32_t)aie__align(HW, 16), 16) : 0;
   p->rec_bytes = (int32_t)aie__align(cur, 16);
 
   const int64_t E = p->E;
@@ -849,7 +850,6 @@
   p->a_layout_prob = a;
   if (c->layout_gen != AIE_LAYOUT_FIXED) a = aie__align(a + (int64_t)AIE_N_RES * HW * 8, 256);
   p->layout_stage_stride = (HW + 15) / 16 * 16;
-  p->layout_pad_ = 0;
   p->a_layout_stage = p->a_layout_tag = p->a_layout_ctl = a;
   if (aie__layout_staged(c)) {
     p->a_layout_stage = a; a = aie__align(a + E * p->layout_stage_stride, 256);
@@ -922,6 +922,7 @@
       REC("regen_src_n", AIE_I32, p->o_src_n, 0, 0, 0, 0);
       REC("regen_src_list", AIE_I16, p->o_src_list, 1, AIE_SRC_CAP, 0, 0);
     }
+    if (p->o_cells8) REC("cells_packed", AIE_U8, p->o_cells8, 2, p->H, p->W, 0);
     REC("mt", AIE_U32, p->o_mt, 1, aie__rng_state_words(&p->c), 0, 0);
     REC("mt_pos", AIE_I32, p->o_mt_pos, 0, 0, 0, 0);
     REC("mt_has_gauss", AIE_I32, p->o_mt_has_gauss, 0, 0, 0, 0);
diff --git a/ai-economist_amd/csrc/aie_spec_generated.h b/ai-economist_amd/csrc/aie_spec_generated.h
--- a/ai-economist_amd/csrc/aie_spec_generated.h
+++ b/ai-economist_amd/csrc/aie_spec_generated.h
@@ -130,7 +130,7 @@
   50,0,0,0,7,0,0,0,21,0,0,0,148,0,0,0,21,0,0,0,1,0,0,0,7,0,0,0,136,0,0,0,
   86,0,0,0,8,0,0,0,0,0,0,0,2,0,0,0,114,0,0,0,115,0,0,0,130,0,0,0,131,0,0,0,
   0,0,0,0,68,0,0,0,82,0,0,0,83,0,0,0,0,0,0,0,3,0,0,0,0,0,0,0,50,0,0,0,
-  154,0,0,0,144,27,0,0,0,0,0,0,176,10,0,0,192,10,0,0,208,10,0,0,240,10,0,0,200,9,0,0,
+  154,0,0,0,16,30,0,0,0,0,0,0,176,10,0,0,192,10,0,0,208,10,0,0,240,10,0,0,200,9,0,0,
   232,9,0,0,8,10,0,0,40,10,0,0,72,10,0,0,104,10,0,0,136,10,0,0,208,13,0,0,216,13,0,0,
   224,13,0,0,128,14,0,0,32,15,0,0,64,15,0,0,152,15,0,0,16,11,0,0,88,16,0,0,96,16,0,0,
   240,15,0,0,16,16,0,0,48,16,0,0,80,16,0,0,124,16,0,0,128,16,0,0,132,16,0,0,156,16,0,0,
@@ -168,7 +168,7 @@
   90,90,90,90,90,90,90,90,90,90,90,90,90,90,90,90,90,90,90,90,90,90,90,90,90,90,90,90,90,90,90,90,
   90,90,90,90,90,90,90,90,90,90,90,90,90,90,90,90,0,0,0,0,0,0,0,0,0,0,0,0,0,0,0,0,
   0,0,0,0,0,0,0,0,0,0,0,0,0,0,0,0,0,0,0,0,0,0,0,0,0,0,0,0,0,0,0,0,
-  0,0,0,0,0,0,0,0,0,0,0,0,0,0,0,0,128,2,0,0,0,0,0,0,0,0,0,0,0,0,0,0,
+  0,0,0,0,0,0,0,0,0,0,0,0,0,0,0,0,128,2,0,0,144,27,0,0,0,0,0,0,0,0,0,0,
   0,0,0,0,0,0,0,0,90,90,90,90,90,90,90,90,90,90,90,90,90,90,90,90,90,90,90,90,90,90,90,90,
   90,90,90,90,90,90,90,90,90,90,90,90,90,90,90,90,90,90,90,90,90,90,90,90,90,90,90,90,90,90,90,90,
   90,90,90,90,90,90,90,90,90,90,90,90,90,90,90,90,90,90,90,90,90,90,90,90,90,90,90,90,90,90,90,90,
@@ -967,7 +967,7 @@
   6,0,0,0,0,0,0,0,0,0,0,0,1,0,0,0,0,0,0,0,1,0,0,0,1,0,0,0,9,0,0,0,
   4,0,0,0,5,0,0,0,0,0,0,0,2,0,0,0,2,0,0,0,3,0,0,0,3,0,0,0,4,0,0,0,
   0,0,0,0,0,0,0,0,0,0,0,0,1,0,0,0,0,0,0,0,0,0,0,0,0,0,0,0,6,0,0,0,
-  1,0,0,0,240,15,0,0,0,0,0,0,112,4,0,0,128,4,0,0,144,4,0,0,176,4,0,0,136,3,0,0,
+  1,0,0,0,224,16,0,0,0,0,0,0,112,4,0,0,128,4,0,0,144,4,0,0,176,4,0,0,136,3,0,0,
   168,3,0,0,200,3,0,0,232,3,0,0,8,4,0,0,40,4,0,0,72,4,0,0,0,0,0,0,0,0,0,0,
   0,0,0,0,0,0,0,0,0,0,0,0,0,0,0,0,0,0,0,0,0,0,0,0,0,0,0,0,0,0,0,0,
   0,0,0,0,0,0,0,0,0,0,0,0,0,0,0,0,208,4,0,0,212,4,0,0,216,4,0,0,240,4,0,0,
@@ -1005,7 +1005,7 @@
   90,90,90,90,90,90,90,90,90,90,90,90,90,90,90,90,90,90,90,90,90,90,90,90,90,90,90,90,90,90,90,90,
   90,90,90,90,90,90,90,90,90,90,90,90,90,90,90,90,0,0,0,0,0,0,0,0,0,0,0,0,0,0,0,0,
   0,0,0,0,0,0,0,0,0,0,0,0,0,0,0,0,0,0,0,0,0,0,0,0,0,0,0,0,0,0,0,0,
-  0,0,0,0,0,0,0,0,0,0,0,0,0,0,0,0,240,0,0,0,0,0,0,0,0,0,0,0,0,0,0,0,
+  0,0,0,0,0,0,0,0,0,0,0,0,0,0,0,0,240,0,0,0,240,15,0,0,0,0,0,0,0,0,0,0,
   0,0,0,0,0,0,0,0,90,90,90,90,90,90,90,90,90,90,90,90,90,90,90,90,90,90,90,90,90,90,90,90,
   90,90,90,90,90,90,90,90,90,90,90,90,90,90,90,90,90,90,90,90,90,90,90,90,90,90,90,90,90,90,90,90,
   90,90,90,90,90,90,90,90,90,90,90,90,90,90,90,90,90,90,90,90,90,90,90,90,90,90,90,90,90,90,90,90,
@@ -1246,7 +1246,7 @@
   50,0,0,0,7,0,0,0,21,0,0,0,148,0,0,0,21,0,0,0,1,0,0,0,7,0,0,0,136,0,0,0,
   86,0,0,0,6,0,0,0,0,0,0,0,2,0,0,0,114,0,0,0,115,0,0,0,130,0,0,0,131,0,0,0,
   0,0,0,0,68,0,0,0,82,0,0,0,83,0,0,0,0,0,0,0,3,0,0,0,0,0,0,0,50,0,0,0,
-  154,0,0,0,144,27,0,0,0,0,0,0,176,10,0,0,192,10,0,0,208,10,0,0,240,10,0,0,200,9,0,0,
+  154,0,0,0,16,30,0,0,0,0,0,0,176,10,0,0,192,10,0,0,208,10,0,0,240,10,0,0,200,9,0,0,
   232,9,0,0,8,10,0,0,40,10,0,0,72,10,0,0,104,10,0,0,136,10,0,0,208,13,0,0,216,13,0,0,
   224,13,0,0,128,14,0,0,32,15,0,0,64,15,0,0,152,15,0,0,16,11,0,0,88,16,0,0,96,16,0,0,
   240,15,0,0,16,16,0,0,48,16,0,0,80,16,0,0,124,16,0,0,128,16,0,0,132,16,0,0,156,16,0,0,
@@ -1284,7 +1284,7 @@
   90,90,90,90,90,90,90,90,90,90,90,90,90,90,90,90,90,90,90,90,90,90,90,90,90,90,90,90,90,90,90,90,
   90,90,90,90,90,90,90,90,90,90,90,90,90,90,90,90,0,0,0,0,0,0,0,0,0,0,0,0,0,0,0,0,
   0,0,0,0,0,0,0,0,0,0,0,0,0,0,0,0,0,0,0,0,0,0,0,0,0,0,0,0,0,0,0,0,
-  0,0,0,0,0,0,0,0,0,0,0,0,0,0,0,0,128,2,0,0,0,0,0,0,0,0,0,0,0,0,0,0,
+  0,0,0,0,0,0,0,0,0,0,0,0,0,0,0,0,128,2,0,0,144,27,0,0,0,0,0,0,0,0,0,0,
   0,0,0,0,0,0,0,0,90,90,90,90,90,90,90,90,90,90,90,90,90,90,90,90,90,90,90,90,90,90,90,90,
   90,90,90,90,90,90,90,90,90,90,90,90,90,90,90,90,90,90,90,90,90,90,90,90,90,90,90,90,90,90,90,90,
   90,90,90,90,90,90,90,90,90,90,90,90,90,90,90,90,90,90,90,90,90,90,90,90,90,90,90,90,90,90,90,90,
@@ -1525,7 +1525,7 @@
   50,0,0,0,0,0,0,0,0,0,0,0,1,0,0,0,0,0,0,0,1,0,0,0,1,0,0,0,136,0,0,0,
   86,0,0,0,6,0,0,0,0,0,0,0,2,0,0,0,114,0,0,0,115,0,0,0,130,0,0,0,131,0,0,0,
   0,0,0,0,68,0,0,0,82,0,0,0,83,0,0,0,0,0,0,0,3,0,0,0,0,0,0,0,50,0,0,0,
-  1,0,0,0,144,27,0,0,0,0,0,0,176,10,0,0,192,10,0,0,208,10,0,0,240,10,0,0,200,9,0,0,
+  1,0,0,0,16,30,0,0,0,0,0,0,176,10,0,0,192,10,0,0,208,10,0,0,240,10,0,0,200,9,0,0,
   232,9,0,0,8,10,0,0,40,10,0,0,72,10,0,0,104,10,0,0,136,10,0,0,208,13,0,0,216,13,0,0,
   224,13,0,0,128,14,0,0,32,15,0,0,64,15,0,0,152,15,0,0,16,11,0,0,88,16,0,0,96,16,0,0,
   240,15,0,0,16,16,0,0,48,16,0,0,80,16,0,0,124,16,0,0,128,16,0,0,132,16,0,0,156,16,0,0,
@@ -1563,7 +1563,7 @@
   90,90,90,90,90,90,90,90,90,90,90,90,90,90,90,90,90,90,90,90,90,90,90,90,90,90,90,90,90,90,90,90,
   90,90,90,90,90,90,90,90,90,90,90,90,90,90,90,90,0,0,0,0,0,0,0,0,0,0,0,0,0,0,0,0,
   0,0,0,0,0,0,0,0,0,0,0,0,0,0,0,0,0,0,0,0,0,0,0,0,0,0,0,0,0,0,0,0,
-  0,0,0,0,0,0,0,0,0,0,0,0,0,0,0,0,128,2,0,0,0,0,0,0,0,0,0,0,0,0,0,0,
+  0,0,0,0,0,0,0,0,0,0,0,0,0,0,0,0,128,2,0,0,144,27,0,0,0,0,0,0,0,0,0,0,
   0,0,0,0,0,0,0,0,90,90,90,90,90,90,90,90,90,90,90,90,90,90,90,90,90,90,90,90,90,90,90,90,
   90,90,90,90,90,90,90,90,90,90,90,90,90,90,90,90,90,90,90,90,90,90,90,90,90,90,90,90,90,90,90,90,
   90,90,90,90,90,90,90,90,90,90,90,90,90,90,90,90,90,90,90,90,90,90,90,90,90,90,90,90,90,90,90,90,
@@ -1804,7 +1804,7 @@
   50,0,0,0,7,0,0,0,21,0,0,0,148,0,0,0,21,0,0,0,1,0,0,0,7,0,0,0,136,0,0,0,
   86,0,0,0,8,0,0,0,0,0,0,0,2,0,0,0,114,0,0,0,115,0,0,0,130,0,0,0,131,0,0,0,
   0,0,0,0,68,0,0,0,82,0,0,0,83,0,0,0,0,0,0,0,3,0,0,0,0,0,0,0,50,0,0,0,
-  154,0,0,0,208,16,0,0,0,0,0,0,176,10,0,0,192,10,0,0,208,10,0,0,240,10,0,0,200,9,0,0,
+  154,0,0,0,80,19,0,0,0,0,0,0,176,10,0,0,192,10,0,0,208,10,0,0,240,10,0,0,200,9,0,0,
   232,9,0,0,8,10,0,0,40,10,0,0,72,10,0,0,104,10,0,0,136,10,0,0,208,13,0,0,216,13,0,0,
   224,13,0,0,128,14,0,0,32,15,0,0,64,15,0,0,152,15,0,0,16,11,0,0,88,16,0,0,96,16,0,0,
   240,15,0,0,16,16,0,0,48,16,0,0,80,16,0,0,124,16,0,0,128,16,0,0,132,16,0,0,156,16,0,0,
@@ -1842,7 +1842,7 @@
   90,90,90,90,90,90,90,90,90,90,90,90,90,90,90,90,90,90,90,90,90,90,90,90,90,90,90,90,90,90,90,90,
   90,90,90,90,90,90,90,90,90,90,90,90,90,90,90,90,0,0,0,0,0,0,0,0,0,0,0,0,0,0,0,0,
   0,0,0,0,0,0,0,0,0,0,0,0,0,0,0,0,0,0,0,0,0,0,0,0,0,0,0,0,0,0,0,0,
-  0,0,0,0,0,0,0,0,0,0,0,0,0,0,0,0,128,2,0,0,0,0,0,0,0,0,0,0,0,0,0,0,
+  0,0,0,0,0,0,0,0,0,0,0,0,0,0,0,0,128,2,0,0,208,16,0,0,0,0,0,0,0,0,0,0,
   0,0,0,0,0,0,0,0,90,90,90,90,90,90,90,90,90,90,90,90,90,90,90,90,90,90,90,90,90,90,90,90,
   90,90,90,90,90,90,90,90,90,90,90,90,90,90,90,90,90,90,90,90,90,90,90,90,90,90,90,90,90,90,90,90,
   90,90,90,90,90,90,90,90,90,90,90,90,90,90,90,90,90,90,90,90,90,90,90,90,90,90,90,90,90,90,90,90,
@@ -2362,7 +2362,7 @@
   6,0,0,0,0,0,0,0,0,0,0,0,1,0,0,0,0,0,0,0,1,0,0,0,1,0,0,0,9,0,0,0,
   4,0,0,0,5,0,0,0,0,0,0,0,2,0,0,0,2,0,0,0,3,0,0,0,3,0,0,0,4,0,0,0,
   0,0,0,0,0,0,0,0,0,0,0,0,1,0,0,0,0,0,0,0,0,0,0,0,0,0,0,0,6,0,0,0,
-  1,0,0,0,64,6,0,0,0,0,0,0,112,4,0,0,128,4,0,0,144,4,0,0,176,4,0,0,136,3,0,0,
+  1,0,0,0,48,7,0,0,0,0,0,0,112,4,0,0,128,4,0,0,144,4,0,0,176,4,0,0,136,3,0,0,
   168,3,0,0,200,3,0,0,232,3,0,0,8,4,0,0,40,4,0,0,72,4,0,0,0,0,0,0,0,0,0,0,
   0,0,0,0,0,0,0,0,0,0,0,0,0,0,0,0,0,0,0,0,0,0,0,0,0,0,0,0,0,0,0,0,
   0,0,0,0,0,0,0,0,0,0,0,0,0,0,0,0,208,4,0,0,212,4,0,0,216,4,0,0,240,4,0,0,
@@ -2400,7 +2400,7 @@
   90,90,90,90,90,90,90,90,90,90,90,90,90,90,90,90,90,90,90,90,90,90,90,90,90,90,90,90,90,90,90,90,
   90,90,90,90,90,90,90,90,90,90,90,90,90,90,90,90,0,0,0,0,0,0,0,0,0,0,0,0,0,0,0,0,
   0,0,0,0,0,0,0,0,0,0,0,0,0,0,0,0,0,0,0,0,0,0,0,0,0,0,0,0,0,0,0,0,
-  0,0,0,0,0,0,0,0,0,0,0,0,0,0,0,0,240,0,0,0,0,0,0,0,0,0,0,0,0,0,0,0,
+  0,0,0,0,0,0,0,0,0,0,0,0,0,0,0,0,240,0,0,0,64,6,0,0,0,0,0,0,0,0,0,0,
   0,0,0,0,0,0,0,0,90,90,90,90,90,90,90,90,90,90,90,90,90,90,90,90,90,90,90,90,90,90,90,90,
   90,90,90,90,90,90,90,90,90,90,90,90,90,90,90,90,90,90,90,90,90,90,90,90,90,90,90,90,90,90,90,90,
   90,90,90,90,90,90,90,90,90,90,90,90,90,90,90,90,90,90,90,90,90,90,90,90,90,90,90,90,90,90,90,90,
```
